# ChainBreak/denoising_diffusion_deep_fake

Measured on AMD Instinct MI355X. Metric: training images/sec (256x256 U-Net, bs=16/GPU), higher is better.
Workload: dtype f32; 1 GPU; d3f train_denoiser step: noise blend -> Unet(resnet34) fwd -> (MSE+1-SSIM)/2 -> bwd -> Adam, 256x256 synthetic face crops, bs=16/GPU, random-init weights, train-mode BatchNorm; image_size=256, batch_per_gpu=16, global_batch=16, parallelism=dp1, graph_step=False, adam_overlap_tail=False, adam_overlap_tail_steps=0, ranks_seen=1, csrc_digest=56899a78a27ce7a0

## Files before the change

### denoising_diffusion_deep_fake_amd/_lib.py

```python
import ctypes as C
import os
import re
from pathlib import Path

_HERE = Path(__file__).resolve().parent
LIB_PATH = Path(os.environ["D3F_LIB"]) if os.environ.get("D3F_LIB") else _HERE / "csrc" / "libd3f_hip.so"
HEADER_PATH = _HERE.parent / "include" / "d3f_hip.h"

F32, BF16, F32X3 = 0, 1, 2


class D3FError(RuntimeError):
    pass


class ConvDesc(C.Structure):
    _fields_ = [(n, C.c_int32) for n in
                ("B", "H", "W", "C0", "C1", "upsample0", "Cout", "KH", "KW", "stride", "pad", "CinReal")]


class BnDesc(C.Structure):
    _fields_ = [("dtype", C.c_int32), ("C", C.c_int32), ("Cpad", C.c_int32), ("rows", C.c_int64),
                ("apply", C.c_int32), ("relu", C.c_int32), ("res", C.c_int32), ("mask", C.c_int32),
                ("fwd_rows", C.c_int32), ("fused_rows", C.c_int32), ("allow_fused", C.c_int32), ("plan_nets", C.c_int32)]


class BnPlan(C.Structure):
    _fields_ = [("fwd_fused", C.c_int32), ("bwd_fused", C.c_int32), ("reduce_blocks", C.c_int32), ("bwd_rows", C.c_int32),
                ("rows_per_block", C.c_int64), ("stat_floats", C.c_uint64), ("part_floats", C.c_uint64)]


BN_COEF_ROWS = 7

_p, _i, _i64, _f, _sz, _dbl = C.c_void_p, C.c_int, C.c_int64, C.c_float, C.c_size_t, C.c_double
_u64, _u32p = C.c_uint64, C.POINTER(C.c_uint32)
_desc = C.POINTER(ConvDesc)
_bnd, _bnp = C.POINTER(BnDesc), C.POINTER(BnPlan)

PROTOTYPES = {
    "d3f_version": (_i, []),
    "d3f_last_error": (C.c_char_p, []),
    "d3f_source_digest": (C.c_char_p, []),
    "d3f_profile_enable": (_i, [_i]),
    "d3f_profile_classes": (_i, [_i]),
    "d3f_profile_collect": (_i, [C.POINTER(C.c_double), C.POINTER(C.c_int64), C.POINTER(C.c_double)]),
    "d3f_unet_create": (_i, [C.c_char_p, _i, _i, _i, _i, _i, _i, C.POINTER(_p)]),
    "d3f_unet_destroy": (_i, [_p]),
    "d3f_unet_create_nets": (_i, [C.c_char_p, _i, _i, _i, _i, _i, _i, _i, _i, C.POINTER(_p)]),
    "d3f_unet_nets": (_i, [_p]),
    "d3f_unet_net_workspace_stride": (_sz, [_p]),
    "d3f_unet_pair_pack_weights": (_i, [_p, C.POINTER(_p), _p, _p]),
    "d3f_unet_pair_forward": (_i, [_p, C.POINTER(_p), C.POINTER(_p), C.POINTER(_p), C.POINTER(_p), _p, _p]),
    "d3f_unet_pair_backward": (_i, [_p, C.POINTER(_p), C.POINTER(_p), C.POINTER(_p), _p, _i, _i, _i, _p]),
    "d3f_unet_num_params": (_i, [_p]),
    "d3f_unet_param_info": (_i, [_p, _i, C.c_char_p, _i, C.POINTER(C.c_int32), C.POINTER(_i), C.POINTER(_i64)]),
    "d3f_unet_param_floats": (_i64, [_p]),
    "d3f_unet_num_bn": (_i, [_p]),
    "d3f_unet_bn_info": (_i, [_p, _i, C.c_char_p, _i, C.POINTER(_i), C.POINTER(_i64), C.POINTER(_i64)]),
    "d3f_unet_bnstat_floats": (_i64, [_p]),
    "d3f_unet_workspace_bytes": (_sz, [_p]),
    "d3f_unet_forward_flops": (_dbl, [_p]),
    "d3f_unet_backward_flops": (_dbl, [_p]),
    "d3f_unet_pack_weights": (_i, [_p, _p, _p, _p]),
    "d3f_unet_forward": (_i, [_p, _p, _p, _p, _p, _p, _i, _p]),
    "d3f_unet_forward_graph": (_i, [_p, _p, _p, _p, _p, _p, _p]),
    "d3f_noise_blend_fixed": (_i, [_p, _p, _p, _p, _i, _i64, _p]),
    "d3f_l1_per_image_workspace_bytes": (_sz, [_i]),
    "d3f_l1_per_image": (_i, [_p, _p, _p, _p, _i, _i64, _p]),
    "d3f_affine_warp": (_i, [_p, _p, _p, _i, _i, _i, _i, _p]),
    "d3f_u8rgb_normalise": (_i, [_p, _p, _i, _i, _i, C.POINTER(_f), C.POINTER(_f), _p]),
    "d3f_unet_predict_u8": (_i, [_p, _p, _p, _p, _p, C.POINTER(_f), C.POINTER(_f), _p, _i, _p]),
    "d3f_unet_predict_frames_u8": (_i, [_p, _p, _p, _p, _i, _i, _i, _i, _i, _i, _p, C.POINTER(_f), C.POINTER(_f), _p, _i, _p]),
    "d3f_crop_resize_cubic_u8": (_i, [_p, _i, _i, _i, _i, _i, _i, _i, _p, _i, _i, _i64, _p]),
    "d3f_unet_num_segments": (_i, [_p]),
    "d3f_unet_plan_counts": (_i, [_p, C.POINTER(C.c_int32), C.POINTER(C.c_int32), C.POINTER(C.c_int32)]),
    "d3f_unet_segment_range": (_i, [_p, _i, C.POINTER(_i64), C.POINTER(_i64)]),
    "d3f_unet_backward": (_i, [_p, _p, _p, _p, _p, _i, _i, _p]),
    "d3f_unet_backward_nojoin": (_i, [_p, _p, _p, _p, _p, _i, _i, _p]),
    "d3f_unet_side_stream": (_i, [_p, C.POINTER(_p)]),
    "d3f_unet_backward_join": (_i, [_p, _p]),
    "d3f_adam_coefficients": (_i, [_f, _f, _f, _f, _i, _f, C.POINTER(_f)]),
    "d3f_unet_train_step": (_i, [_p, _p, _f, _f, _f, _p, _i, _p]),
    "d3f_unet_set_bn_sync": (_i, [_p, _p, _p, _i]),
    "d3f_unet_export": (_i, [_p, C.c_char_p, _p, _p, _p]),
    "d3f_unet_export_shape": (_i, [_p, C.c_char_p, C.POINTER(C.c_int32)]),
    "d3f_conv_upsample_folded": (_i, [_i, _p]),
    "d3f_conv_upsample_summed": (_i, [_i, _p]),
    "d3f_conv_packed_bytes": (_sz, [_i, _desc, _i]),
    "d3f_conv_pack_weights": (_i, [_i, _desc, _p, _p, _p, _p]),
    "d3f_conv_workspace_bytes": (_sz, [_i, _desc, _i]),
    "d3f_conv_stats_floats": (_sz, [_i, _desc, _i, C.POINTER(_i)]),
    "d3f_conv_forward": (_i, [_i, _desc, _p, _p, _p, _p, _p, _p, _p]),
    "d3f_conv_winograd_applies": (_i, [_i, _desc]),
    "d3f_conv_winograd_filter_bytes": (_sz, [_desc]),
    "d3f_conv_winograd_stats_floats": (_sz, [_desc, C.POINTER(_i)]),
    "d3f_conv_winograd_pack": (_i, [_desc, _p, _p, _p]),
    "d3f_conv_winograd_forward": (_i, [_desc, _p, _p, _p, _p, _p, _p, _p, _i, _p]),
    "d3f_conv_backward_data": (_i, [_i, _desc, _p, _p, _p, _p, _i, _i, _p, _p]),
    "d3f_conv_backward_weight_workspace_bytes": (_sz, [_i, _desc]),
    "d3f_conv_backward_weight": (_i, [_i, _desc, _p, _p, _p, _p, _p, _p]),
    "d3f_bn_finalize": (_i, [_p, _i, _i, _i64, _p, _p, _p, _p, _p, _p]),
    "d3f_bn_apply": (_i, [_i, _p, _p, _i, _i64, _p, _i, _p, _p]),
    "d3f_bn_backward_workspace_bytes": (_sz, [_i, _i, _i64]),
    "d3f_bn_backward": (_i, [_i, _p, _p, _p, _p, _p, _i, _i64, _p, _p, _p, _p, _p, _p]),
    "d3f_bn_layer_plan": (_i, [_bnd, _bnp]),
    "d3f_bn_layer_forward": (_i, [_bnd, _p, _p, _p, _p, _p, _p, _p, _p, _p, _p, _p]),
    "d3f_bn_layer_backward": (_i, [_bnd, _p, _p, _p, _p, _p, _p, _p, _p, _i, _p, _p, _p]),
    "d3f_unet_bn_layer": (_i, [_p, _i, _bnd, _bnp]),
    "d3f_maxpool3x3s2_forward": (_i, [_i, _p, _p, _p, _i, _i, _i, _i, _p]),
    "d3f_maxpool3x3s2_backward": (_i, [_i, _p, _p, _p, _i, _i, _i, _i, _i, _p]),
    "d3f_upsample2x_backward": (_i, [_i, _p, _p, _i, _i, _i, _i, _p]),
    "d3f_nchw_to_nhwc": (_i, [_i, _p, _p, _i, _i, _i, _i, _i, _p]),
    "d3f_nhwc_to_nchw": (_i, [_i, _p, _p, _i, _i, _i, _i, _i, _p]),
    "d3f_noise_blend": (_i, [_p, _p, _p, _f, _p, _p, _i, _i64, _p]),
    "d3f_mse_ssim_loss_workspace_bytes": (_sz, [_i, _i, _i]),
    "d3f_mse_ssim_loss": (_i, [_p, _p, _f, _f, _p, _p, _p, _i, _i, _i, _p]),
    "d3f_adam_step": (_i, [_p, _p, _p, _p, _i64, _f, _f, _f, _f, _i, _f, _p]),
    "d3f_ema_lerp": (_i, [_p, _p, _i64, _f, _p]),
    "d3f_philox4x32_10": (_i, [_u32p, _u32p, _u32p]),
    "d3f_noise_blend_rng": (_i, [_p, _u64, _u64, _f, _p, _p, _i, _i64, _p]),
    "d3f_noise_blend_fixed_rng": (_i, [_p, _u64, _u64, _p, _p, _i, _i64, _p]),
    "d3f_noise_draw": (_i, [_u64, _u64, _p, _p, _i, _i64, _p]),
    "d3f_affine_warp_rng": (_i, [_p, _p, _u64, _u64, _i, C.POINTER(_f), _i, _i, _i, _i, _p]),
    "d3f_affine_theta_draw": (_i, [_u64, _u64, _i, C.POINTER(_f), _p, _p, _i, _i, _i, _p]),
}

ALLREDUCE_FN = C.CFUNCTYPE(C.c_int, C.c_void_p, C.c_void_p, C.c_int64, C.c_void_p)

_lib = None


def header_symbols():
    text = HEADER_PATH.read_text()
    text = re.sub(r"/\*.*?\*/", "", text, flags=re.S)
    return sorted(set(re.findall(r"\b(d3f_[a-z0-9_]+)\s*\(", text)))


def sources_present():
    return HEADER_PATH.exists() and any((_HERE / "csrc").glob("*.hip"))


def source_digest():
    import hashlib
    h = hashlib.sha256()
    files = sorted((_HERE / "csrc").glob("*.hip")) + sorted((_HERE / "csrc").glob("*.h")) + [HEADER_PATH]
    for f in files:
        h.update(f.name.encode())
        h.update(f.read_bytes())
    return h.hexdigest()[:16]


def lib():
    global _lib
    if _lib is not None:
        return _lib
    if not LIB_PATH.exists():
        raise D3FError(
            f"{LIB_PATH} is missing: build it with `python -c 'import __graft_entry__ as g; g.build()'` "
            f"or `make -C {LIB_PATH.parent}` (hipcc, gfx950). There is no CPU fallback.")
    handle = C.CDLL(str(LIB_PATH))
    for name, (res, args) in PROTOTYPES.items():
        if os.environ.get("D3F_LIB") and not hasattr(handle, name):
            continue
        fn = getattr(handle, name)
        fn.restype = res
        fn.argtypes = args
    if not os.environ.get("D3F_LIB") and sources_present():
        built, here = handle.d3f_source_digest().decode(), source_digest()
        if built != here:
            raise D3FError(
                f"{LIB_PATH} was built from other sources (digest {built}) than the ones next to it ({here}): "
                f"rebuild it with `make -C {LIB_PATH.parent}`, or name a variant build explicitly through D3F_LIB")
    _lib = handle
    return _lib


def built_digest():
    handle = lib()
    return handle.d3f_source_digest().decode() if hasattr(handle, "d3f_source_digest") else None


def check(rc):
    if rc != 0:
        raise D3FError(lib().d3f_last_error().decode("utf-8", "replace"))


def stream_ptr():
    import torch
    return C.c_void_p(torch.cuda.current_stream().cuda_stream)


def ptr(t):
    if t is None:
        return None
    return C.c_void_p(t.data_ptr())


def ptr2(a, b):
    return (C.c_void_p * 2)(a.data_ptr(), b.data_ptr())
```

### denoising_diffusion_deep_fake_amd/csrc/c_api.hip

```cpp
#include "../../include/d3f_hip.h"

#include <cstdarg>
#include <cstdio>
#include <cstring>
#include <new>
#include <vector>

#include "engine.h"
#include "philox.h"

namespace d3f {
static thread_local char g_err[1024] = "";
int set_error(int code, const char* fmt, ...) {
  va_list ap;
  va_start(ap, fmt);
  vsnprintf(g_err, sizeof(g_err), fmt, ap);
  va_end(ap);
  return code;
}
}

namespace d3f {
struct ProfRec {
  hipEvent_t a, b;
// ... 214 lines not shown
}

int d3f_unet_num_segments(d3f_unet_t h) { return h ? h->e.num_segments : -1; }
int d3f_unet_plan_counts(d3f_unet_t h, int32_t fwd[16], int32_t dgrad[16], int32_t wgrad[16]) {
  D3F_CHECK(h && fwd && dgrad && wgrad, "unet_plan_counts: null argument");
  for (int i = 0; i < 16; ++i) fwd[i] = dgrad[i] = wgrad[i] = 0;
  auto slot = [](int id) { return id < 0 ? 0 : id > 14 ? 14 : id; };
  for (const Unit& u : h->e.units) {
    ++fwd[u.wino ? 15 : slot(u.fwd.patch)];
    if (u.need_dgrad) {
      if (u.upfold) {
        ++dgrad[slot(u.dgrad_lo.patch)];
        if (u.C1 > 0) ++dgrad[slot(u.dgrad.patch)];
      } else {
        ++dgrad[slot(u.dgrad.patch)];
      }
    }
    for (int i = 0; i < u.wl.nparts; ++i) ++wgrad[slot(u.wl.part[i].patch)];
  }
  return 0;
}
int d3f_unet_segment_range(d3f_unet_t h, int segment, int64_t* begin, int64_t* end) {
  D3F_CHECK(h && segment >= 0 && segment < h->e.num_segments, "segment_range: segment %d", segment);
  *begin = h->e.seg_grad_begin[segment];
  *end = h->e.seg_grad_end[segment];
  return 0;
}
int d3f_unet_backward(d3f_unet_t h, const float* params, const float* grad_out, float* grads,
                      void* workspace, int seg_begin, int seg_end, void* stream) {
  D3F_CHECK(h && params && grad_out && grads && workspace, "unet_backward: null argument");
  if (int rc = single_net(h, "unet_backward", "takes d3f_unet_pair_backward")) return rc;
  D3F_CHECK(seg_begin >= 0 && seg_end <= h->e.num_segments && seg_begin <= seg_end,
            "unet_backward: segments [%d,%d)", seg_begin, seg_end);
  return h->e.backward(params, grad_out, grads, workspace, seg_begin, seg_end, (hipStream_t)stream);
}
int d3f_unet_backward_nojoin(d3f_unet_t h, const float* params, const float* grad_out, float* grads,
                             void* workspace, int seg_begin, int seg_end, void* stream) {
  D3F_CHECK(h && params && grad_out && grads && workspace, "unet_backward_nojoin: null argument");
  if (int rc = single_net(h, "unet_backward_nojoin", "takes d3f_unet_pair_backward(join = 0)")) return rc;
  D3F_CHECK(seg_begin >= 0 && seg_end <= h->e.num_segments && seg_begin <= seg_end,
            "unet_backward_nojoin: segments [%d,%d)", seg_begin, seg_end);
  return h->e.backward(params, grad_out, grads, workspace, seg_begin, seg_end, (hipStream_t)stream, 0);
}
int d3f_unet_side_stream(d3f_unet_t h, void** stream_out) {
  D3F_CHECK(h && stream_out, "unet_side_stream: null argument");
  *stream_out = (void*)h->e.side_stream();
  return 0;
}
int d3f_unet_backward_join(d3f_unet_t h, void* stream) {
  D3F_CHECK(h, "unet_backward_join: null handle");
  return h->e.backward_join((hipStream_t)stream);
}
int d3f_adam_coefficients(float lr, float beta1, float beta2, float eps, int step, float grad_scale, float coef[8]) {
  D3F_CHECK(coef && step >= 1, "adam_coefficients: step counts from 1");
  adam_coefficients(lr, beta1, beta2, eps, step, grad_scale, coef);
  return 0;
}
int d3f_unet_train_step(d3f_unet_t h, const d3f_step_buffers* b, float lam, float input_min, float input_max,
                        void* workspace, int use_graph, void* stream) {
  D3F_CHECK(h && b && workspace, "unet_train_step: null argument");
  if (int rc = single_net(h, "unet_train_step", "has no captured step (d3f_unet_pair_forward / _backward, then per network)"))
    return rc;
  D3F_CHECK(b->params && b->bnstats && b->grads && b->exp_avg && b->exp_avg_sq && b->image && b->noise && b->y_uniform &&
                b->noisy && b->pred && b->grad_pred && b->loss_out && b->loss_workspace && b->adam_coef,
            "unet_train_step: null buffer");
  D3F_CHECK(!h->e.bn_sync_installed(),
            "unet_train_step: synchronised BatchNorm statistics call back into the host inside the pass; the captured "
            "step is the single-GPU form (use forward / backward)");
  UnetEngine::StepArgs a;
  std::memset(&a, 0, sizeof(a));
  a.params = b->params; a.bnstats = b->bnstats; a.grads = b->grads; a.exp_avg = b->exp_avg; a.exp_avg_sq = b->exp_avg_sq;
  a.image = b->image; a.noise = b->noise; a.y_uniform = b->y_uniform;
  a.noisy = b->noisy; a.pred = b->pred; a.gpred = b->grad_pred; a.loss_out = b->loss_out;
  a.loss_ws = reinterpret_cast<float*>(b->loss_workspace);
  a.adam_coef = b->adam_coef;
  a.lam = lam; a.lo = input_min; a.hi = input_max;
  return h->e.train_step(a, workspace, use_graph, (hipStream_t)stream);
}
int d3f_unet_set_bn_sync(d3f_unet_t h, d3f_allreduce_fn fn, void* ctx, int world_size) {
  D3F_CHECK(h && (fn == nullptr || world_size >= 1), "unet_set_bn_sync: arguments");
  if (fn != nullptr) {
    if (int rc = single_net(h, "unet_set_bn_sync", "keeps per-GPU BatchNorm statistics")) return rc;
  }
  h->e.set_bn_sync(fn, ctx, world_size);
  return 0;
}
int d3f_unet_export(d3f_unet_t h, const char* name, const void* workspace, float* out_nchw, void* stream) {
  D3F_CHECK(h && name && workspace && out_nchw, "unet_export: null argument");
  return h->e.export_tensor(name, workspace, out_nchw, (hipStream_t)stream);
}
int d3f_unet_export_shape(d3f_unet_t h, const char* name, int32_t dims[3]) {
  D3F_CHECK(h && name && dims, "unet_export_shape: null argument");
  return h->e.export_shape(name, dims);
}

size_t d3f_conv_packed_bytes(int dtype, const d3f_conv_desc* d, int which) {
  ConvLayer L;
  if (plan(L, dtype, d, 0) != 0) return 0;
  if (L.upfold) return which == 0 ? L.wfc : L.wd4 + L.wds;
  return which == 0 ? L.wf : L.wd;
}
int d3f_conv_pack_weights(int dtype, const d3f_conv_desc* d, const float* w, void* w_fwd, void* w_dgrad,
                          void* stream) {
  ConvLayer L;
  if (int rc = plan(L, dtype, d, 0)) return rc;
  if (L.upfold) {
    D3F_CHECK(w_fwd != nullptr && d->CinReal == d->C0 + d->C1, "conv_pack_weights: up-sample folded layer");
    char* wds = w_dgrad && d->C1 > 0 ? reinterpret_cast<char*>(w_dgrad) + L.wd4 : nullptr;
    return pack_up_launch(dtype, w, d->Cout, d->C0, d->C1, w_fwd, L.CoutPad, w_dgrad, L.C0Rows, wds, L.C1Rows,
                          (hipStream_t)stream);
  }
  void* const dst[2] = {w_fwd, w_dgrad};
  PackTable t[2];
  int blocks[2] = {0, 0};
  for (int k = 0; k < 2; ++k) {
    t[k].n = dst[k] != nullptr ? 1 : 0;
    if (t[k].n && (blocks[k] = conv_pack_entry(L, 0, 0, 0, k == 0, k == 1, 0, t[k].e[0])) < 0) return blocks[k];
  }
  for (int k = 0; k < 2; ++k)
    if (int rc = pack_all_launch(dtype, w, dst[k], t[k], blocks[k], (hipStream_t)stream)) return rc;
  return 0;
}
int d3f_conv_upsample_folded(int dtype, const d3f_conv_desc* d) {
  ConvLayer L;
  return (d != nullptr && plan(L, dtype, d, 0) == 0 && L.upfold) ? 1 : 0;
}
int d3f_conv_upsample_summed(int dtype, const d3f_conv_desc* d) {
  ConvLayer L, D;
  if (d == nullptr || !d->upsample0 || plan(L, dtype, d, 0) != 0 || L.upfold) return 0;
  return (plan(D, dtype, d, PLAN_DGRAD | PLAN_SUM2) == 0 && D.dgrad.sum2) ? 1 : 0;
}
size_t d3f_conv_workspace_bytes(int dtype, const d3f_conv_desc* d, int which) {
  ConvLayer L;
  const int what = which == 0 ? PLAN_FWD : PLAN_DGRAD | (d != nullptr && d->upsample0 == 2 ? PLAN_SUM2 : 0);
  return plan(L, dtype, d, what | PLAN_SPLITK) != 0 ? 0 : L.splitk_floats * sizeof(float);
}
size_t d3f_conv_stats_floats(int dtype, const d3f_conv_desc* d, int with_workspace, int* tiles) {
  ConvLayer L;
  if (plan(L, dtype, d, PLAN_FWD | (with_workspace ? PLAN_SPLITK : 0)) != 0) return 0;
  if (tiles) *tiles = L.fwd.stat_rows;
  return (size_t)L.fwd.stat_rows * L.CoutPad * 2;
}
int d3f_conv_forward(int dtype, const d3f_conv_desc* d, const void* src0, const void* src1,
                     const void* w_fwd, void* y, float* stats, void* workspace, void* stream) {
  ConvLayer L;
  if (int rc = plan(L, dtype, d, PLAN_FWD | (workspace ? PLAN_SPLITK : 0))) return rc;
  if (d->B == 0) return 0;
  D3F_CHECK(src0 && w_fwd && y && (d->C1 == 0 || src1), "conv_forward: null argument");
  ConvFwdBufs b;
  b.src0 = src0; b.src1 = src1; b.w = w_fwd; b.out = y; b.stats = stats;
  b.slabs = reinterpret_cast<float*>(workspace);
  return conv_layer_forward(L, b, false, (hipStream_t)stream);
}
static int wino_plan(ConvLayer& L, const d3f_conv_desc* d) {
  if (int rc = plan(L, D3F_F32, d, PLAN_FWD)) return rc;
  D3F_CHECK(L.wu != 0,
            "conv_winograd: needs 3x3 / stride 1 / pad 1, one source, H and W multiples of 16, channels a multiple of 16, "
            "filters a multiple of 64 (got %dx%d k%d s%d p%d C0=%d C1=%d up=%d Cout=%d)",
            d->H, d->W, d->KH, d->stride, d->pad, d->C0, d->C1, d->upsample0, d->Cout);
  return 0;
}
int d3f_conv_winograd_applies(int dtype, const d3f_conv_desc* d) {
  ConvLayer L;
  return (d != nullptr && plan(L, dtype, d, PLAN_FWD) == 0 && L.wino) ? 1 : 0;
}
size_t d3f_conv_winograd_filter_bytes(const d3f_conv_desc* d) {
  ConvLayer L;
  return (d == nullptr || plan(L, D3F_F32, d, PLAN_FWD) != 0) ? 0 : L.wu;
}
size_t d3f_conv_winograd_stats_floats(const d3f_conv_desc* d, int* tiles) {
  ConvLayer L;
  if (d == nullptr || plan(L, D3F_F32, d, PLAN_FWD) != 0 || L.wu == 0) return 0;
  if (tiles) *tiles = L.wino_rows;
  return (size_t)L.wino_rows * L.CoutPad * 2;
}
int d3f_conv_winograd_pack(const d3f_conv_desc* d, const float* w, void* u, void* stream) {
  ConvLayer L;
  if (int rc = wino_plan(L, d)) return rc;
  D3F_CHECK(w && u && d->CinReal == d->C0, "conv_winograd_pack: null argument or padded input channels");
  return conv_winograd_pack_launch(w, reinterpret_cast<float*>(u), d->Cout, d->C0, (hipStream_t)stream);
}
int d3f_conv_winograd_forward(const d3f_conv_desc* d, const void* src0, const void* u, void* y, float* stats,
                              const float* scale, const float* shift, const void* residual, int relu, void* stream) {
  ConvLayer L;
  if (int rc = wino_plan(L, d)) return rc;
  if (d->B == 0) return 0;
  D3F_CHECK(src0 && u && y && ((scale == nullptr) == (shift == nullptr)), "conv_winograd_forward: null argument");
  D3F_CHECK(scale != nullptr || (residual == nullptr && relu == 0),
            "conv_winograd_forward: residual / ReLU belong to the eval epilogue (scale and shift)");
  ConvFwdBufs b;
  b.src0 = src0; b.w = u; b.out = y;
  if (scale != nullptr) {
    b.scale = scale; b.shift = shift; b.res = residual; b.relu = relu ? 1 : 0;
  } else {
    b.stats = stats;
  }
  return conv_layer_forward(L, b, true, (hipStream_t)stream);
}
int d3f_conv_backward_data(int dtype, const d3f_conv_desc* d, const void* dy, const void* w_dgrad,
                           void* dx0, void* dx1, int acc0, int acc1, void* workspace, void* stream) {
  ConvLayer L;
  const int sum2 = d != nullptr && d->upsample0 == 2 ? PLAN_SUM2 : 0;
  if (int rc = plan(L, dtype, d, PLAN_DGRAD | sum2 | (workspace ? PLAN_SPLITK : 0))) return rc;
  if (d->B == 0) return 0;
  D3F_CHECK(dy && w_dgrad && dx0 && (d->C1 == 0 || dx1), "conv_backward_data: null argument");
  ConvDgradBufs b;
  b.dy = dy; b.w = w_dgrad; b.dx0 = dx0; b.dx1 = dx1; b.acc0 = acc0; b.acc1 = acc1;
  b.w_skip = L.upfold ? reinterpret_cast<const char*>(w_dgrad) + L.wd4 : nullptr;
  b.slabs = reinterpret_cast<float*>(workspace);
  return conv_layer_dgrad(L, b, (hipStream_t)stream);
}
size_t d3f_conv_backward_weight_workspace_bytes(int dtype, const d3f_conv_desc* d) {
  ConvLayer L;
  return plan(L, dtype, d, PLAN_WGRAD) != 0 ? 0 : L.wslab_bytes;
}
int d3f_conv_backward_weight(int dtype, const d3f_conv_desc* d, const void* dy, const void* src0,
                             const void* src1, void* workspace, float* dw, void* stream) {
  ConvLayer L;
  if (int rc = plan(L, dtype, d, PLAN_WGRAD)) return rc;
  if (d->B == 0) {
    D3F_CHECK(dw, "conv_backward_weight: null argument");
    D3F_HIP(hipMemsetAsync(dw, 0, (size_t)d->Cout * d->CinReal * d->KH * d->KW * sizeof(float), (hipStream_t)stream));
    return 0;
  }
  D3F_CHECK(dy && src0 && workspace && dw && (d->C1 == 0 || src1), "conv_backward_weight: null argument");
  return wgrad_layer_launch(L.wl, dy, src0, src1, reinterpret_cast<float*>(workspace), dw, d->Cout, d->CinReal, dtype,
                            (hipStream_t)stream);
}

static BnLayer bn_layer(int dtype, int C, int64_t rows, int fwd_rows = 0) {
  BnLayer L;
  L.C = C; L.Cpad = (int)round_up(C, 16); L.rows = (long)rows; L.dtype = sdt(dtype); L.fwd_rows = fwd_rows;
  L.allow_fused = false;
  bn_layer_plan(L);
  return L;
}
int d3f_bn_finalize(const float* stats, int tiles, int C, int64_t count, const float* gamma,
                    const float* beta, float* running_mean, float* running_var, float* coef, void* stream) {
  D3F_CHECK(stats && gamma && beta && coef && C > 0 && tiles > 0 && count > 0, "bn_finalize: argument");
  const BnLayer L = bn_layer(D3F_F32, C, count, tiles);
  BnBufs b;
  b.stats = const_cast<float*>(stats);
  b.gamma = gamma; b.beta = beta; b.running_mean = running_mean; b.running_var = running_var; b.coef = coef;
  return bn_layer_finalize(L, b, (long)count, (hipStream_t)stream);
}
int d3f_bn_apply(int dtype, const void* y, const float* coef, int C, int64_t rows, const void* residual,
                 int relu, void* out, void* stream) {
  D3F_CHECK(y && coef && out, "bn_apply: null argument");
  BnLayer L = bn_layer(dtype, C, rows);
  L.relu = relu != 0;
  L.res = residual ? BN_RES_TENSOR : BN_RES_NONE;
  BnBufs b;
  b.coef = const_cast<float*>(coef);
  b.y = y; b.res = residual; b.a = out;
  return bn_layer_apply(L, b, (hipStream_t)stream);
}
size_t d3f_bn_backward_workspace_bytes(int dtype, int C, int64_t rows) {
  return ((size_t)bn_layer(dtype, C, rows).reduce_blocks * C * 2 + 3 * (size_t)C) * sizeof(float) + 256;
}
int d3f_bn_backward(int dtype, const void* dA, const void* a_or_null, const void* y, const float* coef,
                    const float* gamma, int C, int64_t rows, void* dy, void* dres, float* dgamma,
                    float* dbeta, void* workspace, void* stream) {
  D3F_CHECK(dA && y && coef && gamma && dy && dgamma && dbeta && workspace, "bn_backward: null argument");
  BnLayer L = bn_layer(dtype, C, rows);
  L.mask = a_or_null ? BN_MASK_FROM_A : BN_MASK_NONE;
  BnBufs b;
  b.stats = reinterpret_cast<float*>(workspace);
  b.k = b.stats + (size_t)round_up((long)L.reduce_blocks * C * 2, 4);
  b.coef = const_cast<float*>(coef);
  b.gamma = gamma; b.y = y; b.a = const_cast<void*>(a_or_null);
  b.dA = dA; b.dy = dy; b.dres = dres; b.dgamma = dgamma; b.dbeta = dbeta;
  return bn_layer_backward(L, b, nullptr, (hipStream_t)stream);
}

static_assert(D3F_BN_COEF_ROWS == BN_COEF_ROWS, "d3f_hip.h states the coefficient block's rows");
static int bn_plan(BnLayer& L, const d3f_bn_desc* d) {
  D3F_CHECK(d != nullptr, "bn_layer: null descriptor");
  D3F_CHECK(d->dtype == D3F_F32 || d->dtype == D3F_BF16 || d->dtype == D3F_F32X3, "bn_layer: dtype %d", d->dtype);
  D3F_CHECK(d->C > 0 && d->Cpad >= d->C && d->rows >= 0, "bn_layer: C=%d Cpad=%d rows=%lld", d->C, d->Cpad,
            (long long)d->rows);
  D3F_CHECK(d->res >= BN_RES_NONE && d->res <= BN_RES_LAYER && d->mask >= BN_MASK_NONE && d->mask <= BN_MASK_FROM_A,
            "bn_layer: res=%d mask=%d", d->res, d->mask);
  D3F_CHECK(d->fwd_rows >= 0 && d->fused_rows >= 0, "bn_layer: fwd_rows=%d fused_rows=%d", d->fwd_rows, d->fused_rows);
  D3F_CHECK(d->plan_nets == 1 || d->plan_nets == 2, "bn_layer: plan_nets=%d", d->plan_nets);
  L.name = "bn_layer";
  L.C = d->C; L.Cpad = d->Cpad; L.rows = (long)d->rows; L.dtype = sdt(d->dtype); L.plan_nets = d->plan_nets;
  L.apply = d->apply != 0; L.relu = d->relu != 0;
  L.res = (BnResidual)d->res; L.mask = (BnMask)d->mask;
  L.fwd_rows = d->fwd_rows; L.fused_rows = d->fused_rows; L.allow_fused = d->allow_fused != 0;
  bn_layer_plan(L);
  return 0;
}
static void bn_plan_out(const BnLayer& L, d3f_bn_plan* p) {
  p->fwd_fused = L.fwd_fused; p->bwd_fused = L.bwd_fused; p->reduce_blocks = L.reduce_blocks; p->bwd_rows = L.bwd_rows;
  p->rows_per_block = L.rows_per_block; p->stat_floats = L.stat_floats; p->part_floats = L.part_floats;
}
static bool bn_split_channels_ok(const BnLayer& L) {
  const int ve = L.dtype == D3F_F32 ? 4 : 8;
  return L.C % ve == 0 && (256 * ve) % L.C == 0;
}
int d3f_bn_layer_plan(const d3f_bn_desc* d, d3f_bn_plan* plan) {
  D3F_CHECK(plan != nullptr, "bn_layer_plan: null argument");
  BnLayer L;
  if (int rc = bn_plan(L, d)) return rc;
  bn_plan_out(L, plan);
  return 0;
}
int d3f_bn_layer_forward(const d3f_bn_desc* d, float* stats, const float* gamma, const float* beta, float* running_mean,
                         float* running_var, float* coef, const void* y, const void* res, const float* res_coef, void* a,
                         void* stream) {
  BnLayer L;
  if (int rc = bn_plan(L, d)) return rc;
  if (L.rows == 0) return 0;
  D3F_CHECK(L.fwd_rows >= 1, "bn_layer_forward: the forward pass reads fwd_rows >= 1 partial rows (fwd_rows=%d)", L.fwd_rows);
  D3F_CHECK(stats && gamma && beta && coef && y, "bn_layer_forward: null argument");
  D3F_CHECK((running_mean == nullptr) == (running_var == nullptr), "bn_layer_forward: one running statistic without the other");
  if (L.apply) {
    D3F_CHECK(a != nullptr, "bn_layer_forward: apply needs the output tensor");
    D3F_CHECK(L.res == BN_RES_NONE || res != nullptr, "bn_layer_forward: res=%d needs the residual tensor", (int)L.res);
    D3F_CHECK(L.res != BN_RES_LAYER || res_coef != nullptr, "bn_layer_forward: res=2 needs res_coef, the other layer's coefficient block");
  }
  if (L.fwd_fused)
    D3F_CHECK(L.Cpad % 2 == 0, "bn_layer_forward: the fused form needs an even Cpad (Cpad=%d)", L.Cpad);
  else if (L.apply)
    D3F_CHECK(bn_split_channels_ok(L), "bn_layer_forward: the split form needs C to divide %d (C=%d)",
              256 * (L.dtype == D3F_F32 ? 4 : 8), L.C);
  BnBufs b;
  b.stats = stats; b.gamma = gamma; b.beta = beta; b.running_mean = running_mean; b.running_var = running_var;
  b.coef = coef; b.y = y; b.a = a; b.res = res; b.res_coef = res_coef;
  return bn_layer_forward(L, b, nullptr, (hipStream_t)stream);
}
int d3f_bn_layer_backward(const d3f_bn_desc* d, float* partial, const float* gamma, float* coef, const void* y,
                          const void* a, const void* dA, void* dy, void* dres, int dres_acc, float* dgamma, float* dbeta,
                          void* stream) {
  BnLayer L;
  if (int rc = bn_plan(L, d)) return rc;
  if (L.rows == 0) return 0;
  D3F_CHECK(partial != nullptr, "bn_layer_backward: null partial rows (fused_rows=%d: %s)", L.fused_rows,
            L.fused_rows > 0 ? "the caller's sums" : "scratch of part_floats floats");
  D3F_CHECK(gamma && coef && y && dA && dy, "bn_layer_backward: null argument");
  D3F_CHECK(L.mask != BN_MASK_FROM_A || a != nullptr, "bn_layer_backward: mask=2 needs the activation a");
  D3F_CHECK((dgamma == nullptr) == (dbeta == nullptr), "bn_layer_backward: dgamma without dbeta or the reverse");
  if (L.fused_rows == 0 || !L.bwd_fused)
    D3F_CHECK(bn_split_channels_ok(L), "bn_layer_backward: the split kernels need C to divide %d (C=%d)",
              256 * (L.dtype == D3F_F32 ? 4 : 8), L.C);
  BnBufs b;
  b.stats = partial; b.gamma = gamma; b.coef = coef; b.y = y;
  b.a = const_cast<void*>(a);
  b.dA = dA; b.dy = dy; b.dres = dres; b.dres_acc = dres != nullptr && dres_acc ? 1 : 0;
  b.dgamma = dgamma; b.dbeta = dbeta;
  return bn_layer_backward(L, b, nullptr, (hipStream_t)stream);
}
int d3f_unet_bn_layer(d3f_unet_t h, int i, d3f_bn_desc* d, d3f_bn_plan* plan) {
  D3F_CHECK(h && d && plan && i >= 0 && i < (int)h->e.bns.size(), "bn_layer: index %d", i);
  int k = -1;
  for (const Unit& u : h->e.units) {
    if (!u.bn || ++k != i) continue;
    const BnLayer& L = u.norm;
    d->dtype = L.dtype; d->C = L.C; d->Cpad = L.Cpad; d->rows = L.rows; d->apply = L.apply; d->relu = L.relu;
    d->res = L.res; d->mask = L.mask; d->fwd_rows = L.fwd_rows; d->fused_rows = L.fused_rows;
    d->allow_fused = L.allow_fused; d->plan_nets = L.plan_nets;
    bn_plan_out(L, plan);
// ... 139 lines not shown
```

### denoising_diffusion_deep_fake_amd/csrc/common.h

```cpp
#pragma once
#include <hip/hip_runtime.h>
#include <stdint.h>
#include <stddef.h>
#include <stdlib.h>

namespace d3f {

typedef uint16_t bf16_t;

typedef float f32x16 __attribute__((ext_vector_type(16)));
typedef float f32x4 __attribute__((ext_vector_type(4)));
typedef __bf16 bf16x8 __attribute__((ext_vector_type(8)));

}
#ifndef D3F_F32
#define D3F_F32 0
#define D3F_BF16 1
#define D3F_F32X3 2
#endif
namespace d3f {

static inline const char* prof_knob(const char* name) {
#ifdef D3F_PROFILING
  return getenv(name);
#else
  (void)name;
  return nullptr;
#endif
}

int set_error(int code, const char* fmt, ...);
#define D3F_CHECK(cond, ...)                              \
  do {                                                    \
    if (!(cond)) return ::d3f::set_error(-1, __VA_ARGS__); \
  } while (0)
#define D3F_HIP(expr)                                                                 \
  do {                                                                                \
    hipError_t e_ = (expr);                                                           \
    if (e_ != hipSuccess)                                                             \
      return ::d3f::set_error(-2, "%s failed: %s (%s:%d)", #expr, hipGetErrorString(e_), \
                              __FILE__, __LINE__);                                    \
  } while (0)

__device__ __forceinline__ float bf16_to_f32(bf16_t v) {
  return __uint_as_float(((uint32_t)v) << 16);
}
__device__ __forceinline__ bf16_t f32_to_bf16(float f) {
  __bf16 b = (__bf16)f;
  return *reinterpret_cast<bf16_t*>(&b);
}
template <typename T> __device__ __forceinline__ float to_f32(T v);
template <> __device__ __forceinline__ float to_f32<float>(float v) { return v; }
template <> __device__ __forceinline__ float to_f32<bf16_t>(bf16_t v) { return bf16_to_f32(v); }
template <typename T> __device__ __forceinline__ T from_f32(float v);
template <> __device__ __forceinline__ float from_f32<float>(float v) { return v; }
template <> __device__ __forceinline__ bf16_t from_f32<bf16_t>(float v) { return f32_to_bf16(v); }

template <typename T> __device__ __forceinline__ float4 ld4(const T* p);
template <> __device__ __forceinline__ float4 ld4<float>(const float* p) { return *reinterpret_cast<const float4*>(p); }
template <> __device__ __forceinline__ float4 ld4<bf16_t>(const bf16_t* p) {
  const uint2 v = *reinterpret_cast<const uint2*>(p);
  return make_float4(__uint_as_float(v.x << 16), __uint_as_float(v.x & 0xffff0000u), __uint_as_float(v.y << 16),
                     __uint_as_float(v.y & 0xffff0000u));
}
template <typename T> __device__ __forceinline__ void st4(T* p, const float4& v);
template <> __device__ __forceinline__ void st4<float>(float* p, const float4& v) { *reinterpret_cast<float4*>(p) = v; }
template <> __device__ __forceinline__ void st4<bf16_t>(bf16_t* p, const float4& v) {
  const uint32_t a = (uint32_t)f32_to_bf16(v.x) | ((uint32_t)f32_to_bf16(v.y) << 16);
  const uint32_t b = (uint32_t)f32_to_bf16(v.z) | ((uint32_t)f32_to_bf16(v.w) << 16);
  *reinterpret_cast<uint2*>(p) = make_uint2(a, b);
}

typedef unsigned int u32x4_t __attribute__((ext_vector_type(4)));
constexpr unsigned BUF_OOB = 0x80000000u;
__device__ __forceinline__ __amdgpu_buffer_rsrc_t make_rsrc(const void* p, unsigned bytes) {
  return __builtin_amdgcn_make_buffer_rsrc(const_cast<void*>(p), 0, (int)bytes, 0x00020000);
}
__device__ __forceinline__ uint4 buf_load16(__amdgpu_buffer_rsrc_t r, unsigned byte_off) {
  const u32x4_t v = __builtin_amdgcn_raw_buffer_load_b128(r, (int)byte_off, 0, 0);
  return make_uint4(v.x, v.y, v.z, v.w);
}

__device__ __forceinline__ uint4 buf_load16s(__amdgpu_buffer_rsrc_t r, unsigned byte_off, unsigned soff) {
  const u32x4_t v = __builtin_amdgcn_raw_buffer_load_b128(r, (int)byte_off, (int)soff, 0);
  return make_uint4(v.x, v.y, v.z, v.w);
}

#ifndef D3F_CHAIN_PRIO
#define D3F_CHAIN_PRIO 3
#endif
__device__ __forceinline__ void chain_priority() {
#if D3F_CHAIN_PRIO > 0
  __builtin_amdgcn_s_setprio(D3F_CHAIN_PRIO);
#endif
}

struct NetSplit {
  int nets;
  long ws;
  long par;
  long grad;
  long bn;
  long in;
  long out;
};
static inline int nets_of(int n) { return n > 1 ? n : 1; }
static inline int plan_nets_for(int plan_nets, int bit) {
  static const int mask = prof_knob("D3F_PLAN_MASK") ? atoi(prof_knob("D3F_PLAN_MASK")) : -1;
  return (mask & bit) ? nets_of(plan_nets) : 1;
}
static inline NetSplit net_split_or_single(const NetSplit* ns) {
  NetSplit one{};
  one.nets = 1;
  return (ns != nullptr && ns->nets > 1) ? *ns : one;
}
template <typename P> __device__ __forceinline__ void net_shift(P& p, long bytes) {
  if (p != nullptr) p = reinterpret_cast<P>(reinterpret_cast<uintptr_t>(p) + bytes);
}

template <typename T> struct Elem;
template <> struct Elem<float> {
  static constexpr int VE = 4;
  static constexpr int BKE = 32;
};
template <> struct Elem<bf16_t> {
  static constexpr int VE = 8;
  static constexpr int BKE = 64;
};

static inline void fast_div_setup(unsigned d, unsigned* mul, unsigned* shr) {
  if (d <= 1) { *mul = 0; *shr = 0; return; }
  unsigned lg = 0;
  while ((1ull << lg) < d) ++lg;
  const unsigned p = 31 + lg;
  *mul = (unsigned)(((1ull << p) + d - 1) / d);
  *shr = p - 32;
}
__device__ __forceinline__ int fast_div(int n, unsigned mul, unsigned shr) {
  return mul ? (int)(__umulhi((unsigned)n, mul) >> shr) : n;
}

static inline int cdiv(long a, long b) { return (int)((a + b - 1) / b); }
static inline long round_up(long a, long b) { return (a + b - 1) / b * b; }

enum ProfClass : int { PROF_CONV_FWD = 0, PROF_CONV_DGRAD = 1, PROF_WGRAD = 2, PROF_NUM = 3 };
bool prof_enabled(int cls);
void prof_begin(int cls, double flops, hipStream_t s);
void prof_end(hipStream_t s);

enum ConvMode : int {
  CONV_RAW_STATS = 0,
  CONV_HEAD_NCHW = 1,
  CONV_EVAL_FUSED = 2,
  CONV_DGRAD = 3,
};

struct ConvParams {
  const void* src0;
  const void* src1;
  const void* w;
  void* out0;
  void* out1;
  float* stats;
  const float* scale;
  const float* shift;
  const void* res;
  unsigned src0_bytes, src1_bytes, w_bytes;
  int B, Hv, Wv;
  int C0, C1;
  int H0s, W0s;
  int shift0;
  int zi;
  int Ho, Wo, Cout;
  int CoutPad, Kpad;
  int w_ld;
  int par;
  int nz;
  int KH, KW, stride, pad;
  int M;
  int tiles_m, tiles_n;
  float* partial;
  int splitk;
  int stat_rows;
  int out_c0;
  int acc0, acc1;
  int mode;
  int relu;
  double flops;
  const void* bn_y;
  const float* bn_coef;
  float* bn_partial;
  const void* bn_a;
  unsigned div_howo_mul, div_howo_shr, div_wo_mul, div_wo_shr;
  int cin_real;
  int sum2;
  int patch;
  int nets, plan_nets;
  long net_ws, net_out0, net_scale;
  int tile_bm, tile_bn;
};
__device__ __forceinline__ ConvParams conv_params_of_net(const ConvParams& pin, int net) {
  ConvParams p = pin;
  if (net != 0) {
    net_shift(p.src0, p.net_ws); net_shift(p.src1, p.net_ws); net_shift(p.w, p.net_ws);
    net_shift(p.out0, p.net_out0); net_shift(p.out1, p.net_ws);
    net_shift(p.stats, p.net_ws); net_shift(p.scale, p.net_scale); net_shift(p.shift, p.net_ws);
    net_shift(p.res, p.net_ws); net_shift(p.partial, p.net_ws);
    net_shift(p.bn_y, p.net_ws); net_shift(p.bn_coef, p.net_ws); net_shift(p.bn_partial, p.net_ws); net_shift(p.bn_a, p.net_ws);
  }
  return p;
}

struct ConvTile {
  int BM, BN;
};
int conv_igemm_plan(ConvParams& p, int dtype, bool allow_splitk = false);
size_t conv_splitk_floats(const ConvParams& p);
int conv_igemm_launch(const ConvParams& p, int dtype, hipStream_t stream);
bool conv_winograd_fits(const ConvParams& p, int dtype);
bool conv_winograd_applies(const ConvParams& p, int dtype);
int conv_winograd_stat_rows(const ConvParams& p);
size_t conv_winograd_filter_floats(const ConvParams& p);
int conv_winograd_pack_launch(const float* w , float* u, int Cout, int Cin, hipStream_t stream);
int conv_winograd_launch(const ConvParams& p , hipStream_t stream);
bool conv_pres_applies(const ConvParams& p, int dtype);
void conv_pres_plan(ConvParams& p);
int conv_pres_launch(const ConvParams& p, hipStream_t stream);
bool conv_patch_applies(const ConvParams& p, int dtype);
bool conv_stem_applies(const ConvParams& p, int dtype);
bool conv_stem_bf16_applies(const ConvParams& p, int dtype);
void conv_patch_plan(ConvParams& p, int dtype);
int conv_patch_launch(const ConvParams& p, hipStream_t stream);

struct WgradParams {
  const void* dy;
  const void* src0;
  const void* src1;
  float* partial;
  unsigned dy_bytes, src0_bytes, src1_bytes;
  int B, Hv, Wv, C0, C1, H0s, W0s, shift0;
  int Ho, Wo, Cout;
  int KH, KW, stride, pad;
  int M;
  int cin_real;
  int splits;
  int chunks_per_split;
  int tiles_co, tiles_ci;
  int patch;
  double flops;
  int part;
  int cls;
  int ci_base;
  int slab_cin;
  int slab_taps;
  int Mi, Hc, Wc;
  int step_img, step_row, step_col;
  int nets, plan_nets;
  long net_ws;
};
__device__ __forceinline__ WgradParams wgrad_params_of_net(const WgradParams& pin, int net) {
  WgradParams p = pin;
  if (net != 0) {
    net_shift(p.dy, p.net_ws); net_shift(p.src0, p.net_ws); net_shift(p.src1, p.net_ws); net_shift(p.partial, p.net_ws);
  }
  return p;
}
enum WgradPart : int { WG_WHOLE = 0, WG_CLASS = 1, WG_SKIP = 2 };
int wgrad_plan(WgradParams& p, int dtype);
size_t wgrad_partial_floats(const WgradParams& p);
int wgrad_launch(const WgradParams& p, int dtype, hipStream_t stream);

constexpr int WG_BATCH = 20;
struct WgradReduceJob {
  const float* partial;
  float* dw;
  int splits, CoutP, Cin, CinReal, taps, CB, nsg, VB, CinTot, c_off, fold, Cout, cz, block0, lds;
};
struct WgradReduceBatch {
  WgradReduceJob job[WG_BATCH];
  int n = 0, blocks = 0, lds = 0;
  int nets = 1;
  long net_ws = 0, net_grad = 0;
};
int wgrad_reduce_batch_add(WgradReduceBatch& tb, const float* partial, int splits, int CoutP, int Cout, int Cin,
                           int CinRealPart, int CinRealTotal, int c_off, int KH, int KW, int fold, float* dw);
int wgrad_reduce_batch_launch(const WgradReduceBatch& tb, hipStream_t stream);

struct WgradLayer {
  WgradParams part[2];
  int nparts;
};
int wgrad_layer_plan(WgradLayer& L, const WgradParams& base, int dtype);
size_t wgrad_layer_partial_floats(const WgradLayer& L);
int wgrad_layer_launch(const WgradLayer& L, const void* dy, const void* src0, const void* src1, float* partial,
                       float* dw, int CoutReal, int CinReal, int dtype, hipStream_t stream);
int wgrad_layer_launch_deferred(const WgradLayer& L, const void* dy, const void* src0, const void* src1, float* partial,
                                float* dw, int CoutReal, int CinReal, int dtype, WgradReduceBatch& tb,
                                hipStream_t stream, const NetSplit* ns = nullptr);

struct ConvLayer {
  int B = 0, Hv = 0, Wv = 0;
  int C0 = 0, C1 = 0, up0 = 0;
  int CinReal = 0, Cout = 0, KH = 0, KW = 0, stride = 1, pad = 0;
  int dtype = 0;
  bool head = false;
  bool need_fwd = false, need_dgrad = false, need_wgrad = false;
  bool want_sum2 = false;
  bool allow_splitk = false;
  int plan_nets = 0;
  int sdtype = 0;
  int Cin = 0, Ho = 0, Wo = 0, CoutPad = 0, Kpad = 0, CoutD = 0, KpadD = 0, CinRows = 0, C0Rows = 0, C1Rows = 0;
  bool upfold = false;
  bool parity = false;
  bool wino = false;
  ConvParams fwd{}, dgrad{}, dgrad_lo{};
  WgradLayer wl{};
  int wino_rows = 0;
  size_t wf = 0, wd = 0;
  size_t wfc = 0, wd4 = 0, wds = 0;
  size_t wu = 0;
  size_t splitk_floats = 0;
  size_t wslab_bytes = 0;
  double macs = 0;
};
int conv_layer_plan(ConvLayer& L);

struct ConvFwdBufs {
  const void* src0 = nullptr;
  const void* src1 = nullptr;
  const void* w = nullptr;
  void* out = nullptr;
  float* stats = nullptr;
  const float* bias = nullptr;
  const float* scale = nullptr;
  const float* shift = nullptr;
  const void* res = nullptr;
  int relu = 0;
  float* slabs = nullptr;
};
int conv_layer_forward(const ConvLayer& L, const ConvFwdBufs& b, bool wino, hipStream_t s, const NetSplit* ns = nullptr);
struct ConvDgradBufs {
  const void* dy = nullptr;
  const void* w = nullptr;
  const void* w_skip = nullptr;
  void* dx0 = nullptr;
  void* dx1 = nullptr;
  int acc0 = 0, acc1 = 0;
  float* slabs = nullptr;
  const void* bn_y = nullptr;
  const float* bn_coef = nullptr;
  float* bn_partial = nullptr;
  const void* bn_a = nullptr;
};
int conv_layer_dgrad(const ConvLayer& L, const ConvDgradBufs& b, hipStream_t s, const NetSplit* ns = nullptr);
struct PackEntry;
int conv_pack_entry(const ConvLayer& L, long w_off, size_t wf_off, size_t wd_off, bool fwd, bool dgrad, uint32_t block0,
                    PackEntry& e);

}
```

### denoising_diffusion_deep_fake_amd/csrc/conv_patch.hip

```cpp
#include "common.h"

#include <cstdlib>

namespace d3f {

constexpr int CP_PH = 4, CP_PW = 64;

static bool patch_conv_off() {
  static const bool off = getenv("D3F_NO_PATCH_CONV") != nullptr;
  return off;
}

bool conv_patch_applies(const ConvParams& p, int dtype) {
  if (patch_conv_off() || (dtype != D3F_F32 && dtype != D3F_BF16)) return false;
  const bool mode_ok = p.mode == CONV_RAW_STATS || p.mode == CONV_HEAD_NCHW ||
                       (p.mode == CONV_EVAL_FUSED && p.res == nullptr) ||
                       (p.mode == CONV_DGRAD && p.out_c0 == p.Cout && (p.Cout % 4) == 0);
  const bool wide = p.C0 == 32 && dtype == D3F_BF16 && p.mode != CONV_HEAD_NCHW;
  const bool cin_ok = p.C0 == 16 || wide || (p.C0 == 4 && p.mode == CONV_DGRAD && dtype == D3F_F32) ||
                      (p.C0 == 8 && p.mode == CONV_DGRAD && dtype == D3F_BF16);
  const bool up = wide && p.shift0 == 1 && p.mode != CONV_DGRAD && p.Cout <= 16 && p.H0s * 2 == p.Hv && p.W0s * 2 == p.Wv;
  const bool sum2 = p.sum2 && dtype == D3F_BF16 && p.mode == CONV_DGRAD && p.C0 == 16 && p.Cout == 32 && p.shift0 == 0;
  if (p.sum2 && !sum2) return false;
  return mode_ok && p.par == 0 && p.KH == 3 && p.KW == 3 && p.stride == 1 && p.pad == 1 && cin_ok && p.C1 == 0 &&
         (p.shift0 == 0 || up) && p.zi == 0 && p.Cout <= (wide && !up ? 64 : sum2 ? 32 : 16) && (p.mode == CONV_HEAD_NCHW || (p.Cout % 4) == 0) &&
         p.Hv == p.Ho && p.Wv == p.Wo && (p.Ho % CP_PH) == 0 &&
         (p.Wo % CP_PW) == 0 && p.Kpad >= 9 * p.C0;
}

template <typename T, int CIN, int BN, bool UP = false, int CSRC = CIN, bool SUM2 = false>
__global__ __launch_bounds__(256) void conv_patch_kernel(const ConvParams pin) {
  const ConvParams p = conv_params_of_net(pin, (int)blockIdx.z);
  chain_priority();
  constexpr bool BF = sizeof(T) == 2;
  constexpr bool W64 = BF && CIN == 32;
  static_assert(!UP || (W64 && BN == 16), "up-sampled source: bf16 x 32 channels -> 16 filters");
  static_assert(CSRC == CIN || (BF && CIN == 16 && CSRC == 8 && !UP), "half-filled pixels: bf16, 8 of 16 channels");
  static_assert(!SUM2 || (BF && CIN == 16 && CSRC == 16 && BN == 32 && !UP), "2x2-summed data gradient: bf16 x 16 -> 32");
  static_assert(((CIN == 16 || (CIN == 4 && !BF)) && (BN == 16 || SUM2)) || (W64 && (BN == 32 || UP)),
                "16 channels (forward / data gradient of decoder block 4, head forward), fp32 x 4 (data gradient of the "
                "head) or bf16 x 32 -> 32 (decoder block 3 conv2)");
  constexpr int VEC = 16 / (int)sizeof(T);
  constexpr int PH = CP_PH, PW = CP_PW, PR = UP ? PH / 2 + 2 : PH + 2, PC = UP ? PW / 2 + 2 : PW + 2;
  constexpr int CS = W64 ? 20 : BF ? 10 : (CIN == 16 ? CIN + 4 : 12);
  constexpr int KR = 9 * CIN;
  constexpr int WS = W64 ? KR / 2 : BF ? KR / 2 + 2 : (CIN == 16 ? KR : KR + 4);
  constexpr int CV = CSRC / VEC;
  constexpr int KS = 9 * CSRC;
  constexpr int NPV = PR * PC * CV;
  constexpr int NWV = BN * (KS / VEC);
  constexpr int NLP = (NPV + 255) / 256, NLW = (NWV + 255) / 256;
  constexpr int BM = PH * PW, LDC = BN + 4, FM = PW / 16, NB = BN / 16;
  constexpr int PATCH_DW = PR * PC * CS > BM * LDC ? PR * PC * CS : BM * LDC;
  __shared__ __attribute__((aligned(16))) float lds[PATCH_DW + BN * WS];
  float* P = lds;
  float* Wl = lds + PATCH_DW;

  const int tid = threadIdx.x, lane = tid & 63, wave = tid >> 6;
  const int tiles_x = p.Wo / PW, tiles_y = p.Ho / PH;
  const int tile = (int)blockIdx.x;
  const int tx = tile % tiles_x, ty = (tile / tiles_x) % tiles_y, b = tile / (tiles_x * tiles_y);
  const int y0 = ty * PH, x0 = tx * PW;
  const int n0 = (int)blockIdx.y * BN;

  const __amdgpu_buffer_rsrc_t rs = make_rsrc(p.src0, p.src0_bytes);
  const __amdgpu_buffer_rsrc_t rw = make_rsrc(p.w, p.w_bytes);
  uint4 pv[NLP], wv[NLW];
#pragma unroll
  for (int i = 0; i < NLP; ++i) {
    const int id = tid + 256 * i;
    const int pix = id / CV, cv = id - pix * CV;
    const int pr = pix / PC, pc = pix - pr * PC;
    const int gy = (UP ? y0 / 2 : y0) - 1 + pr, gx = (UP ? x0 / 2 : x0) - 1 + pc;
    const int Hs = UP ? p.H0s : p.Hv, Ws = UP ? p.W0s : p.Wv;
    const bool ok = id < NPV && (unsigned)gy < (unsigned)Hs && (unsigned)gx < (unsigned)Ws;
    pv[i] = buf_load16(rs, ok ? (unsigned)(((b * Hs + gy) * Ws + gx) * CSRC + cv * VEC) * (unsigned)sizeof(T) : BUF_OOB);
  }
#pragma unroll
  for (int i = 0; i < NLW; ++i) {
    const int id = tid + 256 * i;
    const int row = id / (KS / VEC), ch = id - row * (KS / VEC);
    const bool ok = id < NWV && n0 + row < p.CoutPad;
    wv[i] = buf_load16(rw, ok ? (unsigned)((n0 + row) * p.w_ld + ch * VEC) * (unsigned)sizeof(T) : BUF_OOB);
  }
#pragma unroll
  for (int i = 0; i < NLP; ++i) {
    const int id = tid + 256 * i;
    const int pix = id / CV, cv = id - pix * CV;
    if (NPV % 256 == 0 || id < NPV) {
      if constexpr (BF && !W64) {
        *reinterpret_cast<uint2*>(&P[pix * CS + cv * 4]) = make_uint2(pv[i].x, pv[i].y);
        *reinterpret_cast<uint2*>(&P[pix * CS + cv * 4 + 2]) = make_uint2(pv[i].z, pv[i].w);
        if constexpr (CSRC < CIN) {
          *reinterpret_cast<uint2*>(&P[pix * CS + 4]) = make_uint2(0u, 0u);
          *reinterpret_cast<uint2*>(&P[pix * CS + 6]) = make_uint2(0u, 0u);
        }
      } else {
        *reinterpret_cast<uint4*>(&P[pix * CS + cv * 4]) = pv[i];
      }
    }
  }
#pragma unroll
  for (int i = 0; i < NLW; ++i) {
    const int id = tid + 256 * i;
    const int row = id / (KS / VEC), ch = id - row * (KS / VEC);
    if (NWV % 256 == 0 || id < NWV) {
      if constexpr (CSRC < CIN) {
        *reinterpret_cast<uint2*>(&Wl[row * WS + ch * 8]) = make_uint2(wv[i].x, wv[i].y);
        *reinterpret_cast<uint2*>(&Wl[row * WS + ch * 8 + 2]) = make_uint2(wv[i].z, wv[i].w);
        *reinterpret_cast<uint2*>(&Wl[row * WS + ch * 8 + 4]) = make_uint2(0u, 0u);
        *reinterpret_cast<uint2*>(&Wl[row * WS + ch * 8 + 6]) = make_uint2(0u, 0u);
      } else if constexpr (BF && !W64) {
        *reinterpret_cast<uint2*>(&Wl[row * WS + ch * 4]) = make_uint2(wv[i].x, wv[i].y);
        *reinterpret_cast<uint2*>(&Wl[row * WS + ch * 4 + 2]) = make_uint2(wv[i].z, wv[i].w);
      } else {
        const int chs = (CIN == 16 || W64) ? (ch ^ ((row >> 1) & 3)) : ch;
        *reinterpret_cast<uint4*>(&Wl[row * WS + chs * 4]) = wv[i];
      }
    }
  }
  __syncthreads();

  const int fr = lane & 15, fq = lane >> 4;
  f32x4 acc[FM * NB];
#pragma unroll
  for (int i = 0; i < FM * NB; ++i) acc[i] = f32x4{0.f, 0.f, 0.f, 0.f};
  if constexpr (UP) {
    const float* Bbase = Wl + fr * WS + (fq ^ ((fr >> 1) & 3)) * 4;
    const float* Acol[3];
#pragma unroll
    for (int kw = 0; kw < 3; ++kw) Acol[kw] = P + (((fr + kw - 1) >> 1) + 1) * CS + fq * 4;
#pragma unroll
    for (int tap = 0; tap < 9; ++tap) {
      const int kh = tap / 3, kw = tap - kh * 3;
      const int prow = ((wave + kh - 1) >> 1) + 1;
      const uint4 bb = *reinterpret_cast<const uint4*>(Bbase + tap * (CIN / 2));
      uint4 a[FM];
#pragma unroll
      for (int i = 0; i < FM; ++i) a[i] = *reinterpret_cast<const uint4*>(Acol[kw] + (prow * PC + 8 * i) * CS);
#pragma unroll
      for (int i = 0; i < FM; ++i)
        acc[i] = __builtin_amdgcn_mfma_f32_16x16x32_bf16(*reinterpret_cast<const bf16x8*>(&a[i]),
                                                         *reinterpret_cast<const bf16x8*>(&bb), acc[i], 0, 0, 0);
    }
  } else if constexpr (W64) {
    const float* Abase = P + (wave * PC + fr) * CS + fq * 4;
    const float* Bbase = Wl + fr * WS + (fq ^ ((fr >> 1) & 3)) * 4;
#pragma unroll
    for (int tap = 0; tap < 9; ++tap) {
      const int kh = tap / 3, kw = tap - kh * 3;
      uint4 bb[NB], a[FM];
#pragma unroll
      for (int j = 0; j < NB; ++j) bb[j] = *reinterpret_cast<const uint4*>(Bbase + j * 16 * WS + tap * (CIN / 2));
#pragma unroll
      for (int i = 0; i < FM; ++i) a[i] = *reinterpret_cast<const uint4*>(Abase + ((kh * PC + kw) + i * 16) * CS);
#pragma unroll
      for (int i = 0; i < FM; ++i)
#pragma unroll
        for (int j = 0; j < NB; ++j)
          acc[i * NB + j] = __builtin_amdgcn_mfma_f32_16x16x32_bf16(*reinterpret_cast<const bf16x8*>(&a[i]),
                                                                    *reinterpret_cast<const bf16x8*>(&bb[j]), acc[i * NB + j], 0, 0, 0);
    }
  } else if constexpr (BF) {
    typedef short v4s __attribute__((ext_vector_type(4)));
    const float* Abase = P + (wave * PC + fr) * CS + fq * 2;
    const float* Bbase = Wl + fr * WS + fq * 2;
#pragma unroll
    for (int tap = 0; tap < 9; ++tap) {
      const int kh = tap / 3, kw = tap - kh * 3;
      v4s bb[NB];
#pragma unroll
      for (int j = 0; j < NB; ++j) bb[j] = *reinterpret_cast<const v4s*>(Bbase + j * 16 * WS + tap * (CIN / 2));
#pragma unroll
      for (int i = 0; i < FM; ++i) {
        const v4s a = *reinterpret_cast<const v4s*>(Abase + ((kh * PC + kw) + i * 16) * CS);
#pragma unroll
        for (int j = 0; j < NB; ++j) acc[i * NB + j] = __builtin_amdgcn_mfma_f32_16x16x16bf16_1k(a, bb[j], acc[i * NB + j], 0, 0, 0);
      }
    }
  } else if constexpr (CIN == 16) {
    const float* Abase = P + (wave * PC + fr) * CS + fq * 4;
    const float* Bbase = Wl + fr * WS + (fq ^ ((fr >> 1) & 3)) * 4;
#pragma unroll
    for (int tap = 0; tap < 9; ++tap) {
      const int kh = tap / 3, kw = tap - kh * 3;
      const uint4 bb = *reinterpret_cast<const uint4*>(Bbase + tap * CIN);
      uint4 a[FM];
#pragma unroll
      for (int i = 0; i < FM; ++i)
        a[i] = *reinterpret_cast<const uint4*>(Abase + ((kh * PC + kw) + i * 16) * CS);
#pragma unroll
      for (int i = 0; i < FM; ++i) acc[i] = __builtin_amdgcn_mfma_f32_16x16x4f32(__uint_as_float(a[i].x), __uint_as_float(bb.x), acc[i], 0, 0, 0);
#pragma unroll
      for (int i = 0; i < FM; ++i) acc[i] = __builtin_amdgcn_mfma_f32_16x16x4f32(__uint_as_float(a[i].y), __uint_as_float(bb.y), acc[i], 0, 0, 0);
#pragma unroll
      for (int i = 0; i < FM; ++i) acc[i] = __builtin_amdgcn_mfma_f32_16x16x4f32(__uint_as_float(a[i].z), __uint_as_float(bb.z), acc[i], 0, 0, 0);
#pragma unroll
      for (int i = 0; i < FM; ++i) acc[i] = __builtin_amdgcn_mfma_f32_16x16x4f32(__uint_as_float(a[i].w), __uint_as_float(bb.w), acc[i], 0, 0, 0);
    }
  } else {
    const float* Abase = P + (wave * PC + fr) * CS + fq;
    const float* Bbase = Wl + fr * WS + fq;
#pragma unroll
    for (int tap = 0; tap < 9; ++tap) {
      const int kh = tap / 3, kw = tap - kh * 3;
      const float bb = Bbase[tap * CIN];
      float a[FM];
#pragma unroll
      for (int i = 0; i < FM; ++i) a[i] = Abase[((kh * PC + kw) + i * 16) * CS];
#pragma unroll
      for (int i = 0; i < FM; ++i) acc[i] = __builtin_amdgcn_mfma_f32_16x16x4f32(a[i], bb, acc[i], 0, 0, 0);
    }
  }

  const int HoWo = p.Ho * p.Wo;
  const long mrow0 = ((long)b * p.Ho + y0) * p.Wo + x0;
  if (NB == 1 && p.mode == CONV_HEAD_NCHW) {
    if (fr < p.Cout) {
      float* __restrict__ out = reinterpret_cast<float*>(p.out0);
      const float bias = p.scale ? p.scale[fr] : 0.f;
      float* orow = out + ((long)b * p.Cout + fr) * HoWo + (long)(y0 + wave) * p.Wo + x0 + 4 * fq;
#pragma unroll
      for (int i = 0; i < FM; ++i)
        *reinterpret_cast<float4*>(orow + 16 * i) =
            make_float4(acc[i][0] + bias, acc[i][1] + bias, acc[i][2] + bias, acc[i][3] + bias);
    }
    return;
  }
// ... 89 lines not shown
    if (n_ok) {
#pragma unroll
      for (int i = 0; i < NVEC; ++i) {
        const int row = rv0 + i * RSTEP;
        st4<T>(out + out_row(row) * p.Cout + n, *reinterpret_cast<const float4*>(&Cs[row * LDC + cv * 4]));
      }
    }
    if (p.stats != nullptr) {
      constexpr int NG = 256 / BN;
      const int col = tid % BN, rg = tid / BN;
      float s1 = 0.f, s2 = 0.f;
      for (int row = rg; row < BM; row += NG) {
        const float v = Cs[row * LDC + col];
        s1 += v;
        s2 += v * v;
      }
      __syncthreads();
      float* red = lds;
      red[(rg * BN + col) * 2 + 0] = s1;
      red[(rg * BN + col) * 2 + 1] = s2;
      __syncthreads();
      if (tid < BN) {
        float a1 = 0.f, a2 = 0.f;
#pragma unroll
        for (int g = 0; g < NG; ++g) {
          a1 += red[(g * BN + tid) * 2 + 0];
          a2 += red[(g * BN + tid) * 2 + 1];
        }
        if (n0 + tid < p.CoutPad) {
          p.stats[((long)tile * p.CoutPad + n0 + tid) * 2 + 0] = a1;
          p.stats[((long)tile * p.CoutPad + n0 + tid) * 2 + 1] = a2;
        }
      }
    }
  } else if (p.mode == CONV_EVAL_FUSED) {
    T* __restrict__ out = reinterpret_cast<T*>(p.out0);
    if (n_ok) {
      const float4 sc = *reinterpret_cast<const float4*>(p.scale + n), sf = *reinterpret_cast<const float4*>(p.shift + n);
#pragma unroll
      for (int i = 0; i < NVEC; ++i) {
        const int row = rv0 + i * RSTEP;
        float4 v = *reinterpret_cast<const float4*>(&Cs[row * LDC + cv * 4]);
        v.x = v.x * sc.x + sf.x; v.y = v.y * sc.y + sf.y; v.z = v.z * sc.z + sf.z; v.w = v.w * sc.w + sf.w;
        if (p.relu) { v.x = fmaxf(v.x, 0.f); v.y = fmaxf(v.y, 0.f); v.z = fmaxf(v.z, 0.f); v.w = fmaxf(v.w, 0.f); }
        st4<T>(out + out_row(row) * p.Cout + n, v);
      }
    }
  } else {
    T* __restrict__ o0 = reinterpret_cast<T*>(p.out0);
    if (n_ok) {
#pragma unroll
      for (int i = 0; i < NVEC; ++i) {
        const int row = rv0 + i * RSTEP;
        float4 v = *reinterpret_cast<const float4*>(&Cs[row * LDC + cv * 4]);
        T* dst = o0 + out_row(row) * p.Cout + n;
        if (p.acc0) {
          const float4 o = ld4<T>(dst);
          v.x += o.x; v.y += o.y; v.z += o.z; v.w += o.w;
          if (p.bn_partial != nullptr) *reinterpret_cast<float4*>(&Cs[row * LDC + cv * 4]) = v;
        }
        st4<T>(dst, v);
      }
    }
    if (p.bn_partial != nullptr) {
      const int C = p.Cout;
      const T* __restrict__ yb = reinterpret_cast<const T*>(p.bn_y);
      const T* __restrict__ ab = reinterpret_cast<const T*>(p.bn_a);
      float s1[4] = {0.f, 0.f, 0.f, 0.f}, s2[4] = {0.f, 0.f, 0.f, 0.f};
      if (n_ok) {
        const float4 mu = *reinterpret_cast<const float4*>(p.bn_coef + n), is = *reinterpret_cast<const float4*>(p.bn_coef + C + n);
        const float4 sc = *reinterpret_cast<const float4*>(p.bn_coef + 2 * C + n), sf = *reinterpret_cast<const float4*>(p.bn_coef + 3 * C + n);
        const float m4[4] = {mu.x, mu.y, mu.z, mu.w}, i4[4] = {is.x, is.y, is.z, is.w};
        const float c4[4] = {sc.x, sc.y, sc.z, sc.w}, f4[4] = {sf.x, sf.y, sf.z, sf.w};
        float4 yv[NVEC], av[NVEC];
#pragma unroll
        for (int i = 0; i < NVEC; ++i) {
          const long m = out_row(rv0 + i * RSTEP);
          yv[i] = ld4<T>(yb + m * C + n);
          av[i] = ab != nullptr ? ld4<T>(ab + m * C + n) : make_float4(0.f, 0.f, 0.f, 0.f);
        }
#pragma unroll
        for (int i = 0; i < NVEC; ++i) {
          const float4 gv = *reinterpret_cast<const float4*>(&Cs[(rv0 + i * RSTEP) * LDC + cv * 4]);
          const float yy[4] = {yv[i].x, yv[i].y, yv[i].z, yv[i].w}, aa[4] = {av[i].x, av[i].y, av[i].z, av[i].w};
          const float gg[4] = {gv.x, gv.y, gv.z, gv.w};
#pragma unroll
          for (int k = 0; k < 4; ++k) {
            const float keep = ab != nullptr ? aa[k] : yy[k] * c4[k] + f4[k];
            const float g = keep > 0.f ? gg[k] : 0.f;
            s1[k] += g;
            s2[k] += g * ((yy[k] - m4[k]) * i4[k]);
          }
        }
      }
      __syncthreads();
      float* red = lds;
#pragma unroll
      for (int k = 0; k < 4; ++k) {
        red[(rv0 * BN + cv * 4 + k) * 2 + 0] = s1[k];
        red[(rv0 * BN + cv * 4 + k) * 2 + 1] = s2[k];
      }
      __syncthreads();
      if (tid < BN) {
        float a1 = 0.f, a2 = 0.f;
#pragma unroll 8
        for (int g = 0; g < RSTEP; ++g) {
          a1 += red[(g * BN + tid) * 2 + 0];
          a2 += red[(g * BN + tid) * 2 + 1];
        }
        if (n0 + tid < C) {
          p.bn_partial[((long)tile * C + n0 + tid) * 2 + 0] = a1;
          p.bn_partial[((long)tile * C + n0 + tid) * 2 + 1] = a2;
        }
      }
    }
  }
}

constexpr int ST_PH = 8, ST_PW = 32, ST_BN = 32;

bool conv_stem_applies(const ConvParams& p, int dtype) {
  if (patch_conv_off() || dtype != D3F_F32) return false;
  const bool mode_ok = (p.mode == CONV_RAW_STATS) || (p.mode == CONV_EVAL_FUSED && p.res == nullptr);
  return mode_ok && p.par == 0 && p.KH == 7 && p.KW == 7 && p.stride == 2 && p.pad == 3 && p.C0 == 4 && p.C1 == 0 &&
         p.shift0 == 0 && p.zi == 0 && (p.Cout % ST_BN) == 0 && p.Hv == 2 * p.Ho && p.Wv == 2 * p.Wo &&
         (p.Ho % ST_PH) == 0 && (p.Wo % ST_PW) == 0 && p.Kpad >= 49 * 4;
}

__global__ __launch_bounds__(256) void conv_stem_kernel(const ConvParams pin) {
  const ConvParams p = conv_params_of_net(pin, (int)blockIdx.z);
  chain_priority();
  constexpr int PH = ST_PH, PW = ST_PW, BN = ST_BN;
  constexpr int PR = 2 * PH + 5, PC = 2 * PW + 5;
  constexpr int NE = (PC + 1) / 2;
  constexpr int PATCH_DW = PR * PC * 4 + 4;
  constexpr int WS = 7 * 4 * 2 * 4 + 4;
  constexpr int NPV = PR * PC, NWV = BN * 56;
  constexpr int NLP = (NPV + 255) / 256, NLW = (NWV + 255) / 256;
  constexpr int BM = PH * PW, LDC = BN + 4;
  static_assert(BM * LDC <= PATCH_DW + BN * WS, "the C tile aliases the staging area");
  __shared__ __attribute__((aligned(16))) float lds[PATCH_DW + BN * WS];
  float* P = lds;
  float* Wl = lds + PATCH_DW;

  const int tid = threadIdx.x, lane = tid & 63, wave = tid >> 6;
  const int tiles_x = p.Wo / PW, tiles_y = p.Ho / PH;
  const int tile = (int)blockIdx.x, n0 = (int)blockIdx.y * BN;
  const int tx = tile % tiles_x, ty = (tile / tiles_x) % tiles_y, b = tile / (tiles_x * tiles_y);
  const int y0 = ty * PH, x0 = tx * PW;

  const __amdgpu_buffer_rsrc_t rs = make_rsrc(p.src0, p.src0_bytes);
  const __amdgpu_buffer_rsrc_t rw = make_rsrc(p.w, p.w_bytes);
  uint4 pv[NLP], wv[NLW];
#pragma unroll
  for (int i = 0; i < NLP; ++i) {
    const int id = tid + 256 * i;
    const int pr = id / PC, pc = id - pr * PC;
    const int gy = 2 * y0 - 3 + pr, gx = 2 * x0 - 3 + pc;
    const bool ok = id < NPV && (unsigned)gy < (unsigned)p.Hv && (unsigned)gx < (unsigned)p.Wv;
    pv[i] = buf_load16(rs, ok ? (unsigned)(((b * p.Hv + gy) * p.Wv + gx) * 4) * 4u : BUF_OOB);
  }
#pragma unroll
  for (int i = 0; i < NLW; ++i) {
    const int id = tid + 256 * i;
    const int n = id / 56, r = id - n * 56, kh = r >> 3, kw = r & 7;
    const bool ok = id < NWV && kw < 7 && (n0 + n) < p.CoutPad;
    wv[i] = buf_load16(rw, ok ? (unsigned)((n0 + n) * p.w_ld + (kh * 7 + kw) * 4) * 4u : BUF_OOB);
  }
#pragma unroll
  for (int i = 0; i < NLP; ++i) {
    const int id = tid + 256 * i;
    const int pr = id / PC, pc = id - pr * PC;
    if (id < NPV) *reinterpret_cast<uint4*>(&P[(pr * PC + (pc & 1) * NE + (pc >> 1)) * 4]) = pv[i];
  }
  if (tid == 0) *reinterpret_cast<uint4*>(&P[PR * PC * 4]) = make_uint4(0u, 0u, 0u, 0u);
#pragma unroll
  for (int i = 0; i < NLW; ++i) {
    const int id = tid + 256 * i;
    const int n = id / 56, r = id - n * 56;
    if (NWV % 256 == 0 || id < NWV) *reinterpret_cast<uint4*>(&Wl[n * WS + r * 4]) = wv[i];
  }
  __syncthreads();

  const int fr = lane & 31, fq = lane >> 5;
  f32x16 acc[2];
#pragma unroll
  for (int i = 0; i < 2; ++i)
#pragma unroll
    for (int r = 0; r < 16; ++r) acc[i][r] = 0.f;
  const float* Abase = P + ((4 * wave) * PC + fq * NE + fr) * 4;
  const float* Bbase = Wl + fr * WS + fq * 4;
#pragma unroll
  for (int kh = 0; kh < 7; ++kh) {
#pragma unroll
    for (int j = 0; j < 4; ++j) {
      const uint4 bb = *reinterpret_cast<const uint4*>(Bbase + (kh * 4 + j) * 8);
      uint4 a[2];
#pragma unroll
      for (int i = 0; i < 2; ++i) a[i] = *reinterpret_cast<const uint4*>(Abase + ((2 * i + kh) * PC + j) * 4);
#pragma unroll
      for (int i = 0; i < 2; ++i) acc[i] = __builtin_amdgcn_mfma_f32_32x32x2f32(__uint_as_float(a[i].x), __uint_as_float(bb.x), acc[i], 0, 0, 0);
#pragma unroll
      for (int i = 0; i < 2; ++i) acc[i] = __builtin_amdgcn_mfma_f32_32x32x2f32(__uint_as_float(a[i].y), __uint_as_float(bb.y), acc[i], 0, 0, 0);
#pragma unroll
      for (int i = 0; i < 2; ++i) acc[i] = __builtin_amdgcn_mfma_f32_32x32x2f32(__uint_as_float(a[i].z), __uint_as_float(bb.z), acc[i], 0, 0, 0);
    }
  }

  __syncthreads();
  float* Cs = lds;
#pragma unroll
  for (int i = 0; i < 2; ++i)
#pragma unroll
    for (int r = 0; r < 16; ++r)
      Cs[((2 * wave + i) * PW + (r & 3) + 8 * (r >> 2) + 4 * fq) * LDC + fr] = acc[i][r];
  __syncthreads();

  constexpr int VN = BN / 4, NVEC = BM * VN / 256, RSTEP = 256 / VN;
  const int cv = tid % VN, rv0 = tid / VN;
  const int n = n0 + cv * 4;
  const long mrow0 = ((long)b * p.Ho + y0) * p.Wo + x0;
  auto out_row = [&](int row) { return mrow0 + (long)(row / PW) * p.Wo + (row % PW); };
  float* __restrict__ out = reinterpret_cast<float*>(p.out0);
  if (p.mode == CONV_RAW_STATS) {
#pragma unroll
    for (int i = 0; i < NVEC; ++i) {
      const int row = rv0 + i * RSTEP;
      *reinterpret_cast<float4*>(out + out_row(row) * p.Cout + n) = *reinterpret_cast<const float4*>(&Cs[row * LDC + cv * 4]);
    }
    if (p.stats != nullptr) {
      constexpr int NG = 256 / BN;
      const int col = tid % BN, rg = tid / BN;
      float s1 = 0.f, s2 = 0.f;
      for (int row = rg; row < BM; row += NG) {
        const float v = Cs[row * LDC + col];
        s1 += v;
        s2 += v * v;
      }
      __syncthreads();
      float* red = lds;
      red[(rg * BN + col) * 2 + 0] = s1;
      red[(rg * BN + col) * 2 + 1] = s2;
      __syncthreads();
      if (tid < BN) {
        float a1 = 0.f, a2 = 0.f;
#pragma unroll
        for (int g = 0; g < NG; ++g) {
          a1 += red[(g * BN + tid) * 2 + 0];
          a2 += red[(g * BN + tid) * 2 + 1];
        }
        p.stats[((long)tile * p.CoutPad + n0 + tid) * 2 + 0] = a1;
        p.stats[((long)tile * p.CoutPad + n0 + tid) * 2 + 1] = a2;
      }
    }
  } else {
    const float4 sc = *reinterpret_cast<const float4*>(p.scale + n), sf = *reinterpret_cast<const float4*>(p.shift + n);
#pragma unroll
    for (int i = 0; i < NVEC; ++i) {
      const int row = rv0 + i * RSTEP;
      float4 v = *reinterpret_cast<const float4*>(&Cs[row * LDC + cv * 4]);
      v.x = v.x * sc.x + sf.x; v.y = v.y * sc.y + sf.y; v.z = v.z * sc.z + sf.z; v.w = v.w * sc.w + sf.w;
      if (p.relu) { v.x = fmaxf(v.x, 0.f); v.y = fmaxf(v.y, 0.f); v.z = fmaxf(v.z, 0.f); v.w = fmaxf(v.w, 0.f); }
      *reinterpret_cast<float4*>(out + out_row(row) * p.Cout + n) = v;
    }
  }
}

bool conv_stem_bf16_applies(const ConvParams& p, int dtype) {
  if (patch_conv_off() || dtype != D3F_BF16) return false;
#ifdef D3F_NO_PATCH32
  return false;
#endif
  const bool mode_ok = (p.mode == CONV_RAW_STATS) || (p.mode == CONV_EVAL_FUSED && p.res == nullptr);
  return mode_ok && p.par == 0 && p.KH == 7 && p.KW == 7 && p.stride == 2 && p.pad == 3 && p.C0 == 8 && p.C1 == 0 &&
         p.cin_real >= 1 && p.cin_real <= 4 &&
         p.shift0 == 0 && p.zi == 0 && (p.Cout % ST_BN) == 0 && p.Hv == 2 * p.Ho && p.Wv == 2 * p.Wo &&
         (p.Ho % ST_PH) == 0 && (p.Wo % ST_PW) == 0 && p.Kpad >= 49 * 8;
}

__global__ __launch_bounds__(256) void conv_stem_bf16_kernel(const ConvParams pin) {
  const ConvParams p = conv_params_of_net(pin, (int)blockIdx.z);
  chain_priority();
  constexpr int PH = ST_PH, PW = ST_PW, BN = ST_BN;
  constexpr int PR = 2 * PH + 5, PC = 2 * PW + 5;
  constexpr int PCS = PC + 3;
  constexpr int PATCH_DW = PR * PCS * 2 + 4;
  constexpr int WS = 7 * 8 * 2 + 4;
  constexpr int NPV = PR * PC, NWV = BN * 49;
  constexpr int NLP = (NPV + 255) / 256, NLW = (NWV + 255) / 256;
  constexpr int BM = PH * PW, LDC = BN + 4;
  constexpr int LDS_DW = BM * LDC > PATCH_DW + BN * WS ? BM * LDC : PATCH_DW + BN * WS;
  __shared__ __attribute__((aligned(16))) float lds[LDS_DW];
  float* P = lds;
  float* Wl = lds + PATCH_DW;

  const int tid = threadIdx.x, lane = tid & 63, wave = tid >> 6;
  const int tiles_x = p.Wo / PW, tiles_y = p.Ho / PH;
  const int tile = (int)blockIdx.x, n0 = (int)blockIdx.y * BN;
  const int tx = tile % tiles_x, ty = (tile / tiles_x) % tiles_y, b = tile / (tiles_x * tiles_y);
  const int y0 = ty * PH, x0 = tx * PW;

  const __amdgpu_buffer_rsrc_t rs = make_rsrc(p.src0, p.src0_bytes);
  const __amdgpu_buffer_rsrc_t rw = make_rsrc(p.w, p.w_bytes);
  uint4 pv[NLP], wv[NLW];
#pragma unroll
  for (int i = 0; i < NLP; ++i) {
    const int id = tid + 256 * i;
    const int pr = id / PC, pc = id - pr * PC;
    const int gy = 2 * y0 - 3 + pr, gx = 2 * x0 - 3 + pc;
    const bool ok = id < NPV && (unsigned)gy < (unsigned)p.Hv && (unsigned)gx < (unsigned)p.Wv;
    pv[i] = buf_load16(rs, ok ? (unsigned)(((b * p.Hv + gy) * p.Wv + gx) * 8) * 2u : BUF_OOB);
  }
#pragma unroll
  for (int i = 0; i < NLW; ++i) {
    const int id = tid + 256 * i;
    const int n = id / 49, t = id - n * 49;
    const bool ok = id < NWV && (n0 + n) < p.CoutPad;
    wv[i] = buf_load16(rw, ok ? (unsigned)((n0 + n) * p.w_ld + t * 8) * 2u : BUF_OOB);
  }
  for (int id = tid; id < PR * 3; id += 256) {
// ... 152 lines not shown
```

### denoising_diffusion_deep_fake_amd/csrc/conv_plan.hip

```cpp
#include "pointwise.h"

#include <algorithm>

namespace d3f {

int conv_layer_plan(ConvLayer& L) {
  D3F_CHECK(L.dtype == D3F_F32 || L.dtype == D3F_BF16 || L.dtype == D3F_F32X3, "conv: dtype %d", L.dtype);
  L.sdtype = L.dtype == D3F_F32X3 ? D3F_F32 : L.dtype;
  const int ve = L.sdtype == D3F_F32 ? 4 : 8, bke = L.sdtype == D3F_F32 ? 32 : 64;
  const size_t wsz = L.dtype == D3F_F32X3 ? 6 : L.sdtype == D3F_F32 ? 4 : 2;
  D3F_CHECK(L.B >= 0 && L.Hv > 0 && L.Wv > 0 && L.C0 > 0 && L.C1 >= 0 && L.Cout > 0, "conv: extent");
  D3F_CHECK(L.C0 % ve == 0 && L.C1 % ve == 0, "conv: channels must be multiples of %d", ve);
  D3F_CHECK(L.KH == L.KW && L.KH >= 1 && L.KH <= 7, "conv: kernel %dx%d", L.KH, L.KW);
  D3F_CHECK(L.stride == 1 || L.stride == 2, "conv: stride %d", L.stride);
  D3F_CHECK(!L.up0 || (L.Hv % 2 == 0 && L.Wv % 2 == 0), "conv: up-sampled extent must be even");
  D3F_CHECK(L.CinReal > 0 && L.CinReal <= L.C0 + L.C1, "conv: CinReal");

  const int B = L.B, K = L.KH;
  L.Cin = L.C0 + L.C1;
  L.Ho = (L.Hv + 2 * L.pad - K) / L.stride + 1;
  L.Wo = (L.Wv + 2 * L.pad - K) / L.stride + 1;
  L.CoutPad = (int)round_up(L.Cout, 16);
  L.Kpad = (int)round_up((long)K * K * L.Cin, bke);
  L.CoutD = (int)round_up(L.Cout, ve);
  L.KpadD = (int)round_up((long)K * K * L.CoutD, bke);
  L.CinRows = (int)round_up(L.Cin, 16);
  L.C0Rows = (int)round_up(L.C0, 16);
  L.C1Rows = (int)round_up(L.C1, 16);
  L.macs = (double)B * L.Ho * L.Wo * L.Cout * K * K * L.CinReal;
  static const bool no_upfold = prof_knob("D3F_NO_UPFOLD") != nullptr;
  L.upfold = !no_upfold && L.up0 && K == 3 && L.stride == 1 && L.pad == 1 && L.C0 % bke == 0 && L.C1 % bke == 0;
  L.parity = L.stride == 2 && L.C1 == 0 && L.CoutD % bke == 0 && ((K == 3 && L.pad == 1) || (K == 1 && L.pad == 0));
  L.wf = (size_t)L.CoutPad * L.Kpad * wsz;
  L.wd = (size_t)L.CinRows * L.KpadD * wsz;
  if (L.upfold) {
    L.wfc = (size_t)4 * L.CoutPad * (4 * L.C0 + 9 * L.C1) * wsz;
    L.wd4 = (size_t)L.C0Rows * 16 * L.CoutD * wsz;
    L.wds = (size_t)L.C1Rows * L.KpadD * wsz;
  }
  auto plan = [&](ConvParams& p, double flops) {
    p.plan_nets = L.plan_nets;
    p.flops = flops;
    const int rc = conv_igemm_plan(p, L.dtype, L.allow_splitk);
    L.splitk_floats = std::max(L.splitk_floats, conv_splitk_floats(p));
    return rc;
  };

  if (L.need_fwd) {
    ConvParams& f = L.fwd;
    f.B = B; f.Hv = L.Hv; f.Wv = L.Wv; f.C0 = L.C0; f.C1 = L.C1; f.cin_real = L.CinReal;
    f.H0s = L.Hv >> L.up0; f.W0s = L.Wv >> L.up0; f.shift0 = L.up0;
    f.Ho = L.Ho; f.Wo = L.Wo; f.Cout = L.Cout; f.CoutPad = L.CoutPad; f.Kpad = L.Kpad;
    f.KH = f.KW = K; f.stride = L.stride; f.pad = L.pad;
    f.M = B * L.Ho * L.Wo;
    f.mode = L.head ? CONV_HEAD_NCHW : CONV_RAW_STATS;
    if (L.upfold) {
      f.par = 3;
      f.shift0 = 0;
      f.Ho = f.H0s; f.Wo = f.W0s;
      f.M = B * f.H0s * f.W0s;
      f.Kpad = 4 * L.C0 + 9 * L.C1;
    }
    if (int rc = plan(f, 2.0 * L.macs)) return rc;
    L.wino = conv_winograd_applies(f, L.dtype);
    const bool fits = conv_winograd_fits(f, L.dtype);
    L.wino_rows = fits ? conv_winograd_stat_rows(f) : 0;
    L.wu = fits ? conv_winograd_filter_floats(f) * sizeof(float) : 0;
  }

  if (L.need_wgrad) {
    WgradParams g{};
    g.B = B; g.Hv = L.Hv; g.Wv = L.Wv; g.C0 = L.C0; g.C1 = L.C1;
    g.H0s = L.Hv >> L.up0; g.W0s = L.Wv >> L.up0; g.shift0 = L.up0;
    g.Ho = L.Ho; g.Wo = L.Wo; g.Cout = L.CoutD;
    g.KH = g.KW = K; g.stride = L.stride; g.pad = L.pad; g.M = B * L.Ho * L.Wo;
    g.cin_real = L.CinReal;
    g.flops = 2.0 * L.macs;
    g.plan_nets = L.plan_nets;
    if (int rc = wgrad_layer_plan(L.wl, g, L.sdtype)) return rc;
    L.wslab_bytes = wgrad_layer_partial_floats(L.wl) * sizeof(float);
  }

  if (!L.need_dgrad) return 0;
  D3F_CHECK(L.stride == 2 ? (L.Ho * 2 == L.Hv && L.Wo * 2 == L.Wv) : (L.Ho == L.Hv && L.Wo == L.Wv),
            "conv_backward_data: needs a 'same' (stride 1) or exactly halving (stride 2) conv");
  ConvParams dy{};
  dy.B = B; dy.C0 = L.CoutD;
  dy.mode = CONV_DGRAD;
  ConvParams& d = L.dgrad;
  if (L.upfold) {
    ConvParams& l = L.dgrad_lo;
    l = dy;
    l.Hv = l.H0s = L.Hv; l.Wv = l.W0s = L.Wv;
    l.Ho = L.Hv / 2; l.Wo = L.Wv / 2;
    l.Cout = l.out_c0 = L.C0; l.CoutPad = L.C0Rows; l.Kpad = 16 * L.CoutD;
    l.KH = l.KW = 4; l.stride = 2; l.pad = 1;
    l.M = B * l.Ho * l.Wo;
    if (int rc = plan(l, 2.0 * L.macs * L.C0 / L.Cin)) return rc;
    if (L.C1 == 0) return 0;
    d = dy;
    d.Hv = d.H0s = d.Ho = L.Hv; d.Wv = d.W0s = d.Wo = L.Wv;
    d.Cout = d.out_c0 = L.C1; d.CoutPad = L.C1Rows; d.Kpad = L.KpadD;
    d.KH = d.KW = 3; d.stride = 1; d.pad = 1;
    d.M = B * L.Hv * L.Wv;
    return plan(d, 2.0 * L.macs * L.C1 / L.Cin);
  }
  d = dy;
  d.Cout = L.Cin; d.CoutPad = L.CinRows; d.Kpad = L.KpadD;
  d.out_c0 = L.C1 > 0 ? L.C0 : L.Cin;
  if (L.parity) {
    d.par = K == 3 ? 1 : 2;
    d.Hv = d.Ho = d.H0s = L.Ho; d.Wv = d.Wo = d.W0s = L.Wo;
    d.KH = d.KW = K == 3 ? 2 : 1; d.stride = 1; d.pad = 0;
    d.M = B * L.Ho * L.Wo;
  } else {
    const int s2 = L.stride == 2 ? 1 : 0;
    d.Hv = L.Hv; d.Wv = L.Wv;
    d.H0s = L.Ho; d.W0s = L.Wo; d.shift0 = s2; d.zi = s2;
    d.Ho = L.Hv; d.Wo = L.Wv;
    d.KH = d.KW = K; d.stride = 1; d.pad = K - 1 - L.pad;
    d.M = B * L.Hv * L.Wv;
    d.sum2 = (L.want_sum2 && L.up0 && L.C1 == 0) ? 1 : 0;
  }
  return plan(d, 2.0 * L.macs);
}

static void net_conv(ConvParams& p, const NetSplit* ns) {
  if (ns != nullptr) {
    p.nets = ns->nets;
    p.net_ws = p.net_out0 = p.net_scale = ns->ws;
  }
}

int conv_layer_forward(const ConvLayer& L, const ConvFwdBufs& b, bool wino, hipStream_t s, const NetSplit* ns) {
  ConvParams p = L.fwd;
  p.src0 = b.src0; p.src1 = b.src1; p.w = b.w; p.out0 = b.out;
  net_conv(p, ns);
  if (L.head) {
    p.mode = CONV_HEAD_NCHW;
    p.scale = b.bias;
    if (ns != nullptr) {
      p.net_out0 = ns->out;
      p.net_scale = ns->par;
    }
    return conv_igemm_launch(p, L.dtype, s);
  }
  p.partial = p.splitk > 1 ? b.slabs : nullptr;
  if (b.scale != nullptr) {
    p.mode = CONV_EVAL_FUSED;
    p.scale = b.scale; p.shift = b.shift; p.res = b.res; p.relu = b.relu;
  } else {
    p.mode = CONV_RAW_STATS;
    p.stats = b.stats;
    if (wino) p.stat_rows = L.wino_rows;
  }
  return wino ? conv_winograd_launch(p, s) : conv_igemm_launch(p, L.dtype, s);
}

int conv_layer_dgrad(const ConvLayer& L, const ConvDgradBufs& b, hipStream_t s, const NetSplit* ns) {
  ConvParams p = L.upfold ? L.dgrad_lo : L.dgrad;
  p.src0 = b.dy; p.w = b.w; p.out0 = b.dx0; p.acc0 = b.acc0;
  if (!L.upfold) {
    p.out1 = b.dx1;
    p.acc1 = b.acc1;
  }
  p.partial = p.splitk > 1 ? b.slabs : nullptr;
  p.bn_y = b.bn_y; p.bn_coef = b.bn_coef; p.bn_partial = b.bn_partial; p.bn_a = b.bn_a;
  net_conv(p, ns);
  if (p.par == 2 && !p.acc0) {
    const NetSplit nv = net_split_or_single(ns);
    for (int n = 0; n < nv.nets; ++n)
      D3F_HIP(hipMemsetAsync(reinterpret_cast<char*>(b.dx0) + (size_t)n * nv.ws, 0,
                             (size_t)4 * p.M * p.Cout * (L.sdtype == D3F_F32 ? 4 : 2), s));
  }
  if (int rc = conv_igemm_launch(p, L.dtype, s)) return rc;
  if (!L.upfold || L.C1 == 0) return 0;
  ConvParams k = L.dgrad;
  k.src0 = b.dy; k.w = b.w_skip; k.out0 = b.dx1; k.acc0 = b.acc1;
  k.partial = k.splitk > 1 ? b.slabs : nullptr;
  net_conv(k, ns);
  return conv_igemm_launch(k, L.dtype, s);
}

int conv_pack_entry(const ConvLayer& L, long w_off, size_t wf_off, size_t wd_off, bool fwd, bool dgrad, uint32_t block0,
                    PackEntry& e) {
  const int taps = L.KH * L.KW;
  const long nf = fwd ? (long)L.CoutPad * L.Kpad : 0, nd = dgrad ? (long)L.CinRows * L.KpadD : 0;
  D3F_CHECK((!fwd || L.Kpad >= taps * L.Cin) && (!dgrad || L.KpadD >= taps * L.CoutD), "pack_weights: padded K too small");
  const int extent = std::max({L.Cout, L.CinReal, L.Cin, L.CoutPad, L.Kpad, L.CinRows, L.CoutD, L.KpadD});
  D3F_CHECK(extent < 65536 && nf + nd < 0x7fffffffL,
            "pack_weights: the layer exceeds the packing table (extents below 65536, fewer than 2^31 packed elements): "
            "extent %d, %ld elements", extent, nf + nd);
  D3F_CHECK(w_off >= 0 && w_off <= 0xffffffffL && wf_off % 16 == 0 && wd_off % 16 == 0 && (wf_off >> 4) < 0xffffffffull &&
                (wd_off >> 4) < 0xffffffffull,
            "pack_weights: layer out of table range");
  D3F_CHECK(taps <= PACK_LDS_ROW, "pack_weights: %d taps exceed the tile", taps);
  int CT = 32;
  while (CT * taps > PACK_LDS_ROW) CT >>= 1;
  const int crows = std::max(fwd ? L.Cin : 0, dgrad ? L.CinRows : 0);
  const int nrows = std::max(fwd ? L.CoutPad : 0, dgrad ? L.CoutD : 0);
  unsigned mul, shr;
  fast_div_setup((unsigned)taps, &mul, &shr);
  e = PackEntry{};
  e.w_off = (uint32_t)w_off;
  e.wf_off16 = (uint32_t)(wf_off >> 4);
  e.wd_off16 = (uint32_t)(wd_off >> 4);
  e.block0 = block0;
  e.Cout = (uint16_t)L.Cout; e.CinReal = (uint16_t)L.CinReal; e.Cin = (uint16_t)L.Cin;
  e.taps = (uint16_t)taps; e.CoutPad = (uint16_t)L.CoutPad; e.Kpad = (uint16_t)L.Kpad;
  e.CinRows = (uint16_t)L.CinRows; e.CoutD = (uint16_t)L.CoutD; e.KpadD = (uint16_t)L.KpadD;
  e.has_f = fwd ? 1 : 0;
  e.has_d = dgrad ? 1 : 0;
  e.conv_stride = (dgrad && L.parity) ? 2 : 1;
  e.CT = (uint16_t)CT;
  e.ctiles = (uint16_t)((crows + CT - 1) / CT);
  e.taps_mul = mul;
  e.taps_shr = (uint16_t)shr;
  e.ct_log2 = (uint16_t)__builtin_ctz((unsigned)CT);
  return e.ctiles * ((nrows + PACK_NT - 1) / PACK_NT);
}

}
```

### denoising_diffusion_deep_fake_amd/csrc/engine.h

```cpp
#pragma once
#include <string>
#include <vector>

#include "common.h"
#include "pointwise.h"

namespace d3f {

struct TensorD {
  size_t off = 0;
  int H = 0, W = 0, C = 0;
  long elems(int B) const { return (long)B * H * W * C; }
};

struct ParamInfo {
  std::string name;
  int shape[4];
  int ndim;
  long offset;
  long numel;
};

struct BnInfo {
  std::string prefix;
  int C;
  long rm_off, rv_off;
};

struct Unit : ConvLayer {
  std::string conv_name;
  int in0 = -1, in1 = -1, y = -1, a = -1;
  bool bn = true, bias = false;
  BnLayer norm;
  int res_tensor = -1, res_unit = -1;
  long w_off = -1, bias_off = -1, g_off = -1, b_off = -1, rm_off = -1, rv_off = -1;
  size_t wf_off = 0, wd_off = 0;
  size_t coef_off = 0;
  int segment = 0;
  size_t dy_off = 0;
  size_t wfc_off = 0, wd4_off = 0, wds_off = 0;
  size_t wu_off = 0;
  size_t wslab_off = 0;
};

enum BwdKind { BW_HEAD, BW_UNIT, BW_SUM2X2, BW_POOL };
struct BwdOp {
  BwdKind kind;
  int unit = -1;
  int dA = -1;
  int fuse_for_unit = -1;
  int fused_rows = 0;
  bool mask = true;
  int dres = -1;
  bool dres_acc = false;
  int dst0 = -1, dst1 = -1;
  bool acc0 = false, acc1 = false;
  bool dst0_is_full_scratch = false;
  int C = 0, Hl = 0, Wl = 0;
  int segment = 0;
};

struct NetIO {
  long params = 0, bnstats = 0, grads = 0, x = 0, out = 0, dout = 0;
};

class UnetEngine {
 public:
  ~UnetEngine();
  int build(const char* encoder, int in_channels, int classes, int B, int H, int W, int dtype, int nets = 1,
            int plan_nets = 1);

  int pack_weights(const float* params, void* ws, hipStream_t s, const NetIO* io = nullptr) const;
  int forward(const float* params, float* bnstats, const float* x, float* out, void* ws, int training,
              hipStream_t s, const NetIO* io = nullptr) const;
  int backward(const float* params, const float* dout, float* grads, void* ws, int seg_begin,
               int seg_end, hipStream_t s, int join = 1, const NetIO* io = nullptr) const;
  int backward_join(hipStream_t s) const;
  hipStream_t side_stream() const;
  int predict_u8(const float* params, float* bnstats, const uint8_t* bgr_in, uint8_t* bgr_out,
                 const float mean[3], const float stdv[3], void* ws, int use_graph, hipStream_t s) const;
  int predict_frames_u8(const float* params, float* bnstats, const uint8_t* raw_in, int src_h, int src_w, int x1, int y1,
                        int cw, int ch, uint8_t* pair_out, const float mean[3], const float stdv[3], void* ws,
                        int use_graph, hipStream_t s) const;
  int forward_graph(const float* params, float* bnstats, const float* x, float* out, void* ws, hipStream_t s) const;
  struct StepArgs {
    float* params; float* bnstats; float* grads; float* exp_avg; float* exp_avg_sq;
    const float* image; const float* noise; const float* y_uniform;
    float* noisy; float* pred; float* gpred; float* loss_out; float* loss_ws;
    const float* adam_coef;
    float lam, lo, hi;
  };
  int train_step(const StepArgs& a, void* ws, int use_graph, hipStream_t s) const;
  typedef int (*AllReduceFn)(void* ctx, float* data, int64_t count, void* stream);
  bool bn_sync_installed() const { return bn_sync_.fn != nullptr; }
  void set_bn_sync(AllReduceFn fn, void* ctx, int world) { bn_sync_ = BnSync{fn, ctx, world > 0 ? world : 1}; }
  int export_tensor(const char* name, const void* ws, float* out_nchw, hipStream_t s) const;
  int export_shape(const char* name, int32_t dims[3]) const;

  std::vector<ParamInfo> params;
  std::vector<BnInfo> bns;
  long param_floats = 0, bnstat_floats = 0;
  size_t workspace_bytes = 0;
  int num_segments = 4;
  long seg_grad_begin[8] = {0}, seg_grad_end[8] = {0};
  int B = 0, H = 0, W = 0, dtype = 0, in_channels = 3, classes = 3;
  int nets = 1, plan_nets = 1;
  size_t net_ws_stride = 0;
  int cdtype = 0;
  double fwd_flops = 0, bwd_flops = 0;
  std::vector<Unit> units;

 private:
  int esize() const { return dtype == D3F_F32 ? 4 : 2; }
  int wsize() const { return cdtype == D3F_F32X3 ? 6 : esize(); }
  int ve() const { return dtype == D3F_F32 ? 4 : 8; }
  const TensorD* find_export(const char* name) const;
  int new_tensor(int H_, int W_, int C_);
  int new_grad(int tensor_id);
  size_t alloc(size_t bytes);
  int add_unit(const std::string& conv_name, const std::string& bn_name, int in0, int in1, int up0,
               int Cout, int k, int stride, int pad, bool bn, bool bias, bool relu, bool apply,
               int segment);

  std::vector<TensorD> tensors;
  std::vector<TensorD> gtensors;
  std::vector<int> grad_of;
  std::vector<bool> grad_init;
  std::vector<BwdOp> bwd_ops;
  std::vector<int> fwd_order_;
  mutable hipStream_t side_ = nullptr;
  mutable std::vector<hipEvent_t> ev_dy_;
  mutable hipEvent_t ev_join_ = nullptr;
  mutable hipEvent_t ev_seg_ = nullptr;
  mutable bool side_dirty_ = false;
  int ensure_streams() const;
  mutable hipEvent_t ev_pack_in_ = nullptr, ev_pack_done_ = nullptr, ev_pack_mid_ = nullptr;
  mutable bool pack_pending_ = false, pack_mid_pending_ = false;
  int first_mid_unit_ = -1;
  int first_late_unit_ = -1;
  int forward_body(const float* params, float* bnstats, float* out, char* ws, int training, hipStream_t s,
                   const NetSplit* ns = nullptr) const;
  bool make_split(const NetIO* io, long in_delta, NetSplit* ns) const;
  int predict_u8_launches(const float* params, float* bnstats, const uint8_t* bgr_in, uint8_t* bgr_out,
                          const float mean255[3], const float std255[3], char* ws, hipStream_t s) const;
  int predict_frames_u8_launches(const float* params, float* bnstats, const uint8_t* raw_in, const int geo[6],
                                 uint8_t* pair_out, const float mean255[3], const float std255[3], char* ws,
                                 hipStream_t s) const;
  struct GraphKey {
    const void* ptr[5];
    float cst[6];
    int geo[6];
  };
  struct GraphSlot {
    hipGraphExec_t exec = nullptr;
    GraphKey key = {};
  };
  template <typename F>
  int graph_replay(GraphSlot& slot, const GraphKey& key, hipStream_t s, F&& launches) const;
  int wait_for_packed_weights(hipStream_t s) const;
  mutable hipStream_t gstream_ = nullptr;
  mutable GraphSlot g_predict_, g_eval_, g_frames_;
  BnSync bn_sync_{nullptr, nullptr, 1};
  const BnSync* bn_sync() const { return bn_sync_.fn != nullptr ? &bn_sync_ : nullptr; }
  int train_step_launches(const StepArgs& a, void* ws, hipStream_t s) const;
  mutable hipGraphExec_t g_step_ = nullptr;
  mutable StepArgs g_step_key_{};
  mutable const void* g_step_ws_ = nullptr;
  mutable hipEvent_t ev_gin_ = nullptr, ev_gout_ = nullptr;
  size_t head_nchw_off = 0;
  size_t ws_top = 0;
  int t_x = -1, t_pool = -1, head = -1, conv1 = -1;
  size_t pool_idx_off = 0, stats_off = 0, bnpart_off = 0, dz_off = 0, dfull_off = 0,
         bsum_off = 0, splitk_off = 0;
  size_t stats_bytes = 0, bnpart_bytes = 0, dy_bytes = 0, dz_bytes = 0, dfull_bytes = 0, splitk_bytes = 0;
};

int channel_sum_nchw_launch(const float* x, int B, int C, long HW, float* partial, float* out,
                            hipStream_t stream, const NetSplit* ns = nullptr);

}
```

### denoising_diffusion_deep_fake_amd/csrc/engine.hip

```cpp
#include "engine.h"
#include <vector>

#include <cstdio>
#include <cstdlib>
#include <cstring>

namespace d3f {

constexpr int CS_PP = 16;
__global__ __launch_bounds__(256) void channel_sum_partial_kernel(const float* __restrict__ x, int C, long HW,
                                                                  float* __restrict__ partial, int nb, long net_in,
                                                                  long net_ws) {
  __shared__ float red[256];
  const int seg = blockIdx.x, c = blockIdx.y, b = (int)blockIdx.z % nb;
  if ((int)blockIdx.z >= nb) {
    net_shift(x, net_in); net_shift(partial, net_ws);
  }
  const float* __restrict__ plane = x + ((long)b * C + c) * HW;
  const long per = (HW + CS_PP - 1) / CS_PP, lo = (long)seg * per, hi = lo + per < HW ? lo + per : HW;
  float s = 0.f;
  if ((HW & 3) == 0 && (per & 3) == 0) {
    for (long i = lo + 4 * threadIdx.x; i < hi; i += 4 * 256) {
      const float4 v = *reinterpret_cast<const float4*>(plane + i);
      s += (v.x + v.y) + (v.z + v.w);
// ... 245 lines not shown
    op.segment = u.segment;
    if (u.need_dgrad) {
      if (u.upfold) {
        op.dst0 = grad_dst(u.in0, &op.acc0);
        if (u.in1 >= 0) op.dst1 = grad_dst(u.in1, &op.acc1);
        D3F_CHECK(u.segment == 0, "plan: unit %s: a folded up-sampling layer outside the decoder bucket", u.conv_name.c_str());
      } else if (u.up0 && !u.dgrad.sum2) {
        op.dst0_is_full_scratch = true;
        if (u.in1 >= 0) op.dst1 = grad_dst(u.in1, &op.acc1);
      } else {
        op.dst0 = grad_dst(u.in0, &op.acc0);
      }
    }
    bwd_ops.push_back(op);
    if (u.need_dgrad && u.up0 && !u.upfold && !u.dgrad.sum2) {
      BwdOp s;
      s.kind = BW_SUM2X2; s.unit = ui; s.C = u.C0; s.Hl = u.Hv / 2; s.Wl = u.Wv / 2; s.segment = u.segment;
      bool acc;
      s.dst0 = grad_dst(u.in0, &acc);
      D3F_CHECK(!acc, "plan: up-sampled tensor has two consumers");
      bwd_ops.push_back(s);
    }
    return 0;
  };
  {
    BwdOp h;
    h.kind = BW_HEAD; h.unit = head; h.segment = 0;
    h.dst0 = grad_dst(units[head].in0, &h.acc0);
    bwd_ops.push_back(h);
  }
  for (int i = 4; i >= 0; --i) {
    const DBlk& d = dec_blocks[i];
    if (int rc = emit_unit(d.u2, grad_of[units[d.u2].a], true, -1, false)) return rc;
    if (int rc = emit_unit(d.u1, grad_of[units[d.u1].a], true, -1, false)) return rc;
  }
  for (int bi = (int)enc_blocks.size() - 1; bi >= 0; --bi) {
    const Blk& b = enc_blocks[bi];
    const Unit& u2 = units[b.u2];
    D3F_CHECK(grad_of[u2.a] >= 0, "plan: block output without gradient");
    int dres;
    bool dres_acc = false;
    if (b.ud >= 0) dres = -2;
    else dres = grad_dst(u2.res_tensor, &dres_acc);
    if (int rc = emit_unit(b.u2, grad_of[u2.a], true, dres, dres_acc)) return rc;
    if (int rc = emit_unit(b.u1, grad_of[units[b.u1].a], true, -1, false)) return rc;
    if (b.ud >= 0)
      if (int rc = emit_unit(b.ud, -2, false, -1, false)) return rc;
  }
  {
    BwdOp p;
    p.kind = BW_POOL; p.segment = 3;
    p.dA = grad_of[t_pool];
    D3F_CHECK(p.dA >= 0, "plan: pool output without gradient");
    p.dst0 = grad_dst(f1, &p.acc0);
    bwd_ops.push_back(p);
  }
  if (int rc = emit_unit(conv1, grad_of[f1], true, -1, false)) return rc;

  static const bool no_fused_reduce = getenv("D3F_NO_FUSED_BN_REDUCE") != nullptr;
  if (!no_fused_reduce) {
    auto writes = [&](const BwdOp& o, int gid) {
      if (o.kind == BW_UNIT || o.kind == BW_HEAD) {
        if (units[o.unit].need_dgrad && !o.dst0_is_full_scratch && o.dst0 == gid) return true;
        if (o.dst1 == gid) return true;
        if (o.kind == BW_UNIT && o.dres == gid) return true;
      }
      return (o.kind == BW_SUM2X2 || o.kind == BW_POOL) && o.dst0 == gid;
    };
    for (size_t j = 0; j + 1 < bwd_ops.size(); ++j) {
      BwdOp& pj = bwd_ops[j];
      if (!(pj.kind == BW_UNIT || pj.kind == BW_HEAD)) continue;
      const Unit& up = units[pj.unit];
      const ConvParams& pd = up.upfold ? up.dgrad_lo : up.dgrad;
      if (!up.need_dgrad || pd.par || pj.dst0_is_full_scratch || (pj.dst1 >= 0 && !up.upfold) || pj.dst0 < 0) continue;
      BwdOp& ck = bwd_ops[j + 1];
      if (ck.kind != BW_UNIT || ck.dA != pj.dst0) continue;
      bool last = true;
      for (size_t k = j + 1; k < bwd_ops.size(); ++k) last = last && !writes(bwd_ops[k], pj.dst0);
      const Unit& uc = units[ck.unit];
      if (!last || !(uc.bn && ck.mask)) continue;
      D3F_CHECK(pd.Cout == uc.Cout && pd.M == (pd.sum2 ? 4 : 1) * B * uc.Ho * uc.Wo && pd.out_c0 == pd.Cout,
                "plan: fused BatchNorm reduce shape mismatch (%s -> %s)", up.conv_name.c_str(), uc.conv_name.c_str());
      pj.fuse_for_unit = ck.unit;
      ck.fused_rows = pd.splitk > 1 ? pd.stat_rows : pd.tiles_m;
    }
  }

  for (const BwdOp& op : bwd_ops) {
    if (op.kind != BW_UNIT) continue;
    Unit& u = units[op.unit];
    u.norm.res = u.res_tensor >= 0 ? BN_RES_TENSOR : u.res_unit >= 0 ? BN_RES_LAYER : BN_RES_NONE;
    u.norm.mask = !op.mask ? BN_MASK_NONE : u.norm.res == BN_RES_NONE ? BN_MASK_FROM_Y : BN_MASK_FROM_A;
    u.norm.fused_rows = op.fused_rows;
  }
  for (Unit& u : units) {
    if (!u.bn) continue;
    bn_layer_plan(u.norm);
    stats_bytes = std::max(stats_bytes, u.norm.stat_floats * sizeof(float));
    bnpart_bytes = std::max(bnpart_bytes, u.norm.part_floats * sizeof(float));
  }

  stats_off = alloc(stats_bytes);
  bnpart_off = alloc(bnpart_bytes);
  dz_off = alloc(dz_bytes);
  dfull_off = alloc(dfull_bytes);
  bsum_off = alloc(channel_sum_partial_floats(B, classes) * sizeof(float));
  splitk_off = alloc(splitk_bytes);
  head_nchw_off = alloc((size_t)B * classes * H * W * sizeof(float));
  net_ws_stride = nets > 1 ? (size_t)round_up((long)ws_top, 4096) : 0;
  workspace_bytes = nets > 1 ? net_ws_stride * nets : ws_top;

  long layer3_start = -1, layer4_start = -1, dec_start = -1;
  for (const auto& p : params) {
    if (layer3_start < 0 && p.name.rfind("encoder.layer3.", 0) == 0) layer3_start = p.offset;
    if (layer4_start < 0 && p.name.rfind("encoder.layer4.", 0) == 0) layer4_start = p.offset;
    if (dec_start < 0 && p.name.rfind("decoder.", 0) == 0) dec_start = p.offset;
  }
  num_segments = 4;
  seg_grad_begin[0] = dec_start;     seg_grad_end[0] = param_floats;
  seg_grad_begin[1] = layer4_start;  seg_grad_end[1] = dec_start;
  seg_grad_begin[2] = layer3_start;  seg_grad_end[2] = layer4_start;
  seg_grad_begin[3] = 0;             seg_grad_end[3] = layer3_start;
  fwd_order_.clear();
  fwd_order_.push_back(conv1);
  fwd_order_.push_back(-1);
  for (const auto& b : enc_blocks) {
    fwd_order_.push_back(b.u1);
    if (b.ud >= 0) fwd_order_.push_back(b.ud);
    fwd_order_.push_back(b.u2);
  }
  for (const auto& d : dec_blocks) {
    fwd_order_.push_back(d.u1);
    fwd_order_.push_back(d.u2);
  }
  fwd_order_.push_back(head);
  return 0;
}

static int shared_side_stream(hipStream_t* out) {
  constexpr int MAXDEV = 64;
  static hipStream_t streams[MAXDEV] = {};
  int dev = 0;
  D3F_HIP(hipGetDevice(&dev));
  D3F_CHECK(dev >= 0 && dev < MAXDEV, "side stream: device index %d", dev);
  if (streams[dev] == nullptr) {
    int least = 0, greatest = 0;
    D3F_HIP(hipDeviceGetStreamPriorityRange(&least, &greatest));
    D3F_HIP(hipStreamCreateWithPriority(&streams[dev], hipStreamNonBlocking, least));
  }
  *out = streams[dev];
  return 0;
}

int UnetEngine::ensure_streams() const {
  if (side_ != nullptr) return 0;
  if (int rc = shared_side_stream(&side_)) return rc;
  D3F_HIP(hipEventCreateWithFlags(&ev_join_, hipEventDisableTiming));
  D3F_HIP(hipEventCreateWithFlags(&ev_seg_, hipEventDisableTiming));
  D3F_HIP(hipEventCreateWithFlags(&ev_pack_in_, hipEventDisableTiming));
  D3F_HIP(hipEventCreateWithFlags(&ev_pack_done_, hipEventDisableTiming));
  D3F_HIP(hipEventCreateWithFlags(&ev_pack_mid_, hipEventDisableTiming));
  return 0;
}

bool UnetEngine::make_split(const NetIO* io, long in_delta, NetSplit* ns) const {
  if (nets <= 1) return false;
  ns->nets = nets;
  ns->ws = (long)net_ws_stride;
  ns->par = io->params;
  ns->grad = io->grads;
  ns->bn = io->bnstats;
  ns->in = in_delta;
  ns->out = io->out;
  return true;
}

int UnetEngine::pack_weights(const float* params0_, void* ws0_, hipStream_t s, const NetIO* io) const {
  D3F_CHECK((int)units.size() <= PACK_MAX_LAYERS, "pack_weights: %d layers exceed the table", (int)units.size());
  D3F_CHECK(nets == 1 || io != nullptr, "pack_weights: a pair engine needs the second network's offsets");
  static const bool sync_pack = getenv("D3F_NO_ASYNC_PACK") != nullptr;
  const bool async = !sync_pack && first_late_unit_ > 0;
  const int mid = async ? first_mid_unit_ : -1;
  auto params_of = [&](int n) { return reinterpret_cast<const float*>(reinterpret_cast<const char*>(params0_) + (n ? io->params : 0)); };
  auto ws_of = [&](int n) { return reinterpret_cast<char*>(ws0_) + (size_t)n * net_ws_stride; };
  auto part_of = [&](int ui) { return ui >= first_late_unit_ ? 2 : (mid > 0 && ui >= mid) ? 1 : 0; };
  for (int part = 0; part < 3; ++part) {
    if (part == 1 && mid <= 0) continue;
    PackTable t;
    t.n = 0;
    uint32_t blocks = 0;
    for (int ui = 0; ui < (int)units.size(); ++ui) {
      const Unit& u = units[ui];
      if (first_late_unit_ > 0 && part_of(ui) != part) continue;
      if (first_late_unit_ <= 0 && part != 0) continue;
      if (u.upfold) continue;
      const int nb = conv_pack_entry(u, u.w_off, u.wf_off, u.wd_off, true, u.need_dgrad, blocks, t.e[t.n++]);
      if (nb < 0) return nb;
      blocks += (uint32_t)nb;
    }
    hipStream_t ps = s;
    if (part >= 1 && async) {
      if (int rc = ensure_streams()) return rc;
      if (part == 1 || mid <= 0) {
        D3F_HIP(hipEventRecord(ev_pack_in_, s));
        D3F_HIP(hipStreamWaitEvent(side_, ev_pack_in_, 0));
      }
      ps = side_;
    }
    for (int n = 0; n < nets; ++n) {
      const float* params_ = params_of(n);
      char* ws = ws_of(n);
      if (t.n > 0)
        if (int rc = pack_all_launch(cdtype, params_, ws, t, (int)blocks, ps)) return rc;
      for (int ui = 0; ui < (int)units.size(); ++ui) {
        const Unit& u = units[ui];
        if (!u.wino) continue;
        if (first_late_unit_ > 0 ? part_of(ui) != part : part != 0) continue;
        if (int rc = conv_winograd_pack_launch(params_ + u.w_off, reinterpret_cast<float*>(ws + u.wu_off), u.Cout, u.Cin, ps))
          return rc;
      }
    }
    if (part == 1 && async) {
      D3F_HIP(hipEventRecord(ev_pack_mid_, side_));
      pack_mid_pending_ = true;
    }
    if (part == 2 || (first_late_unit_ <= 0 && part == 0)) {
      for (int n = 0; n < nets; ++n) {
        const float* params_ = params_of(n);
        char* ws = ws_of(n);
        for (const Unit& u : units)
          if (u.upfold)
            if (int rc = pack_up_launch(cdtype, params_ + u.w_off, u.Cout, u.C0, u.C1, ws + u.wfc_off, u.CoutPad,
                                        u.need_dgrad ? ws + u.wd4_off : nullptr, u.C0Rows,
                                        (u.need_dgrad && u.C1 > 0) ? ws + u.wds_off : nullptr, u.C1Rows, ps))
              return rc;
      }
    }
    if (part == 2 && async) {
      D3F_HIP(hipEventRecord(ev_pack_done_, side_));
      pack_pending_ = true;
    }
  }
  return 0;
}

int UnetEngine::forward(const float* params_, float* bnstats, const float* x, float* out, void* ws_,
                        int training, hipStream_t s, const NetIO* io) const {
  char* ws = reinterpret_cast<char*>(ws_);
  D3F_CHECK(nets == 1 || (io != nullptr && training), "unet: the pair engine runs train-mode passes and needs the second "
            "network's offsets");
  NetSplit split{};
  const NetSplit* ns = make_split(io, io ? io->x : 0, &split) ? &split : nullptr;
  if (int rc = nchw_to_nhwc_launch(dtype, x, ws + tensors[t_x].off, B, in_channels, H, W, tensors[t_x].C, s, ns))
    return rc;
  return forward_body(params_, bnstats, out, ws, training, s, ns);
}

int UnetEngine::forward_body(const float* params_, float* bnstats, float* out, char* ws, int training,
                             hipStream_t s, const NetSplit* ns) const {
  auto T = [&](int tid) { return ws + tensors[tid].off; };
  auto coef = [&](const Unit& u) { return reinterpret_cast<float*>(ws + u.coef_off); };
  D3F_CHECK(ns == nullptr || (training && bn_sync() == nullptr), "unet: the pair engine runs train-mode passes with "
            "per-GPU BatchNorm statistics");
  if (!training) {
    BnEvalTable t;
    t.n = 0;
    for (const Unit& u : units)
      if (u.bn) {
        D3F_CHECK(t.n < PACK_MAX_LAYERS && u.coef_off % 16 == 0, "eval coefficients: table overflow");
        BnEvalEntry& e = t.e[t.n++];
        e.g_off = (uint32_t)u.g_off; e.b_off = (uint32_t)u.b_off;
        e.rm_off = (uint32_t)u.rm_off; e.rv_off = (uint32_t)u.rv_off;
        e.coef_off16 = (uint32_t)(u.coef_off >> 4);
        e.C = u.Cout;
      }
    if (int rc = bn_eval_coeff_all_launch(params_, bnstats, ws, t, s)) return rc;
  }
  for (int ui : fwd_order_) {
    if (ui < 0) {
      const TensorD& f1 = tensors[units[conv1].a];
      if (int rc = maxpool3x3s2_fwd_launch(dtype, T(units[conv1].a), T(t_pool),
                                           reinterpret_cast<uint8_t*>(ws + pool_idx_off), B, f1.H, f1.W,
                                           f1.C, s, ns))
        return rc;
      continue;
    }
    const Unit& u = units[ui];
    if (pack_mid_pending_ && ui >= first_mid_unit_) {
      D3F_HIP(hipStreamWaitEvent(s, ev_pack_mid_, 0));
      pack_mid_pending_ = false;
    }
    if (pack_pending_ && ui >= first_late_unit_) {
      D3F_HIP(hipStreamWaitEvent(s, ev_pack_done_, 0));
      pack_pending_ = false;
    }
    ConvFwdBufs b;
    b.src0 = T(u.in0);
    b.src1 = u.in1 >= 0 ? T(u.in1) : nullptr;
    b.w = ws + (u.wino ? u.wu_off : u.upfold ? u.wfc_off : u.wf_off);
    b.slabs = reinterpret_cast<float*>(ws + splitk_off);
    if (!u.bn) {
      b.out = out;
      b.bias = params_ + u.bias_off;
      if (int rc = conv_layer_forward(u, b, false, s, ns)) return rc;
      continue;
    }
    const Unit* ds = u.res_unit >= 0 ? &units[u.res_unit] : nullptr;
    if (training) {
      b.out = T(u.y);
      b.stats = reinterpret_cast<float*>(ws + stats_off);
      if (int rc = conv_layer_forward(u, b, u.wino, s, ns)) return rc;
      BnBufs n;
      n.stats = b.stats;
      n.gamma = params_ + u.g_off; n.beta = params_ + u.b_off;
      n.running_mean = bnstats + u.rm_off; n.running_var = bnstats + u.rv_off;
      n.coef = coef(u);
      n.y = T(u.y); n.a = u.a >= 0 ? T(u.a) : nullptr;
      n.res = u.res_tensor >= 0 ? T(u.res_tensor) : (ds ? T(ds->y) : nullptr);
      n.res_coef = ds ? coef(*ds) : nullptr;
      if (int rc = bn_layer_forward(u.norm, n, bn_sync(), s, ns)) return rc;
    } else {
      b.scale = bn_coef(coef(u), u.Cout, BN_SCALE);
      b.shift = bn_coef(coef(u), u.Cout, BN_SHIFT);
      b.relu = u.norm.relu ? 1 : 0;
      if (u.norm.apply) {
        b.out = T(u.a);
        b.res = u.res_tensor >= 0 ? T(u.res_tensor) : (ds ? T(ds->y) : nullptr);
      } else {
        b.out = T(u.y);
      }
      if (int rc = conv_layer_forward(u, b, u.wino, s, ns)) return rc;
    }
  }
  return 0;
}

int UnetEngine::predict_u8_launches(const float* params_, float* bnstats, const uint8_t* bgr_in, uint8_t* bgr_out,
                                    const float mean255[3], const float std255[3], char* ws, hipStream_t s) const {
  if (int rc = u8bgr_to_nhwc_launch(dtype, bgr_in, ws + tensors[t_x].off, (long)B * H * W, tensors[t_x].C, mean255,
                                    std255, s))
    return rc;
  float* head_out = reinterpret_cast<float*>(ws + head_nchw_off);
  if (int rc = forward_body(params_, bnstats, head_out, ws, 0, s)) return rc;
  return nchw_to_u8bgr_launch(head_out, bgr_out, B, H, W, 3L * W, mean255, std255, s);
}

int UnetEngine::predict_u8(const float* params_, float* bnstats, const uint8_t* bgr_in, uint8_t* bgr_out,
                           const float mean[3], const float stdv[3], void* ws_, int use_graph,
                           hipStream_t s) const {
  D3F_CHECK(in_channels == 3 && classes == 3, "predict_u8: 3-channel frames only (in %d, out %d)", in_channels, classes);
  char* ws = reinterpret_cast<char*>(ws_);
  float m255[3], s255[3];
  for (int c = 0; c < 3; ++c) {
    m255[c] = mean[c] * 255.0f;
    s255[c] = stdv[c] * 255.0f;
  }
  if (!use_graph) return predict_u8_launches(params_, bnstats, bgr_in, bgr_out, m255, s255, ws, s);
  const GraphKey key = {{params_, bnstats, bgr_in, bgr_out, ws_}, {m255[0], m255[1], m255[2], s255[0], s255[1], s255[2]}, {}};
  return graph_replay(g_predict_, key, s, [&](hipStream_t gs) {
    return predict_u8_launches(params_, bnstats, bgr_in, bgr_out, m255, s255, ws, gs);
  });
}

int UnetEngine::predict_frames_u8_launches(const float* params_, float* bnstats, const uint8_t* raw_in, const int geo[6],
                                           uint8_t* pair_out, const float mean255[3], const float std255[3], char* ws,
                                           hipStream_t s) const {
  if (int rc = crop_resize_cubic_u8_nhwc_launch(dtype, raw_in, B, geo[0], geo[1], geo[2], geo[3], geo[4], geo[5], pair_out,
                                                H, W, 6L * W, ws + tensors[t_x].off, tensors[t_x].C, mean255, std255, s))
    return rc;
  float* head_out = reinterpret_cast<float*>(ws + head_nchw_off);
  if (int rc = forward_body(params_, bnstats, head_out, ws, 0, s)) return rc;
  return nchw_to_u8bgr_launch(head_out, pair_out + 3L * W, B, H, W, 6L * W, mean255, std255, s);
}

int UnetEngine::predict_frames_u8(const float* params_, float* bnstats, const uint8_t* raw_in, int src_h, int src_w, int x1,
                                  int y1, int cw, int ch, uint8_t* pair_out, const float mean[3], const float stdv[3],
                                  void* ws_, int use_graph, hipStream_t s) const {
  D3F_CHECK(in_channels == 3 && classes == 3, "predict_frames_u8: 3-channel frames only (in %d, out %d)", in_channels,
            classes);
  char* ws = reinterpret_cast<char*>(ws_);
  float m255[3], s255[3];
  for (int c = 0; c < 3; ++c) {
    m255[c] = mean[c] * 255.0f;
    s255[c] = stdv[c] * 255.0f;
  }
  if (int rc = crop_resize_cubic_check(B, src_h, src_w, x1, y1, cw, ch, H, W, 6L * W)) return rc;
  const int geo[6] = {src_h, src_w, x1, y1, cw, ch};
  if (!use_graph) return predict_frames_u8_launches(params_, bnstats, raw_in, geo, pair_out, m255, s255, ws, s);
  const GraphKey key = {{params_, bnstats, raw_in, pair_out, ws_},
                        {m255[0], m255[1], m255[2], s255[0], s255[1], s255[2]},
                        {src_h, src_w, x1, y1, cw, ch}};
  return graph_replay(g_frames_, key, s, [&](hipStream_t gs) {
    return predict_frames_u8_launches(params_, bnstats, raw_in, geo, pair_out, m255, s255, ws, gs);
  });
}

int UnetEngine::forward_graph(const float* params_, float* bnstats, const float* x, float* out, void* ws_,
                              hipStream_t s) const {
  const GraphKey key = {{params_, bnstats, x, out, ws_}, {}, {}};
  return graph_replay(g_eval_, key, s, [&](hipStream_t gs) { return forward(params_, bnstats, x, out, ws_, 0, gs); });
}

int UnetEngine::train_step_launches(const StepArgs& a, void* ws_, hipStream_t s) const {
  const long per_image = (long)in_channels * H * W;
  if (int rc = pack_weights(a.params, ws_, s)) return rc;
  if (int rc = noise_blend_launch(a.image, a.noise, a.y_uniform, a.lam, a.noisy, nullptr, B, per_image, s)) return rc;
  if (int rc = forward(a.params, a.bnstats, a.noisy, a.pred, ws_, 1, s)) return rc;
  if (int rc = mse_ssim_loss_launch(a.pred, a.image, a.lo, a.hi, a.loss_out, a.gpred, a.loss_ws, B, H, W, s)) return rc;
  if (int rc = backward(a.params, a.gpred, a.grads, ws_, 0, num_segments, s, 1)) return rc;
  return adam_step_dev_launch(a.params, a.grads, a.exp_avg, a.exp_avg_sq, param_floats, a.adam_coef, s);
}

int UnetEngine::train_step(const StepArgs& a, void* ws_, int use_graph, hipStream_t s) const {
  D3F_CHECK(in_channels == 3 && classes == 3, "train_step: the (MSE + 1 - SSIM) / 2 objective is defined on 3-channel images");
  if (!use_graph) return train_step_launches(a, ws_, s);
  if (int rc = wait_for_packed_weights(s)) return rc;
  if (int rc = ensure_streams()) return rc;
  if (gstream_ == nullptr) {
    D3F_HIP(hipStreamCreateWithFlags(&gstream_, hipStreamNonBlocking));
    D3F_HIP(hipEventCreateWithFlags(&ev_gin_, hipEventDisableTiming));
    D3F_HIP(hipEventCreateWithFlags(&ev_gout_, hipEventDisableTiming));
  }
  const bool same = g_step_ != nullptr && g_step_ws_ == ws_ && memcmp(&a, &g_step_key_, sizeof(StepArgs)) == 0;
  if (!same) {
    if (g_step_) {
      (void)hipGraphExecDestroy(g_step_);
      g_step_ = nullptr;
    }
    hipGraph_t graph = nullptr;
    D3F_HIP(hipStreamBeginCapture(gstream_, hipStreamCaptureModeThreadLocal));
    const int rc = train_step_launches(a, ws_, gstream_);
    const hipError_t e = hipStreamEndCapture(gstream_, &graph);
    pack_pending_ = pack_mid_pending_ = false;
    side_dirty_ = false;
    if (rc != 0) {
      if (graph) (void)hipGraphDestroy(graph);
      return rc;
    }
    D3F_HIP(e);
    const hipError_t ei = hipGraphInstantiate(&g_step_, graph, nullptr, nullptr, 0);
    (void)hipGraphDestroy(graph);
    D3F_HIP(ei);
    g_step_key_ = a;
    g_step_ws_ = ws_;
  }
  D3F_HIP(hipGraphLaunch(g_step_, s));
  return 0;
}

int UnetEngine::wait_for_packed_weights(hipStream_t s) const {
  if (pack_mid_pending_) {
    D3F_HIP(hipStreamWaitEvent(s, ev_pack_mid_, 0));
    pack_mid_pending_ = false;
  }
  if (pack_pending_) {
    D3F_HIP(hipStreamWaitEvent(s, ev_pack_done_, 0));
    pack_pending_ = false;
  }
  return 0;
}

template <typename F>
int UnetEngine::graph_replay(GraphSlot& slot, const GraphKey& key, hipStream_t s, F&& launches) const {
  if (int rc = wait_for_packed_weights(s)) return rc;
  if (gstream_ == nullptr) {
    D3F_HIP(hipStreamCreateWithFlags(&gstream_, hipStreamNonBlocking));
    D3F_HIP(hipEventCreateWithFlags(&ev_gin_, hipEventDisableTiming));
    D3F_HIP(hipEventCreateWithFlags(&ev_gout_, hipEventDisableTiming));
  }
  static_assert(sizeof(GraphKey) == 5 * sizeof(void*) + 6 * sizeof(float) + 6 * sizeof(int), "GraphKey is compared bytewise");
  const bool same = slot.exec != nullptr && memcmp(&key, &slot.key, sizeof(GraphKey)) == 0;
  if (!same) {
    if (slot.exec) {
      (void)hipGraphExecDestroy(slot.exec);
      slot.exec = nullptr;
    }
    hipGraph_t graph = nullptr;
    D3F_HIP(hipStreamBeginCapture(gstream_, hipStreamCaptureModeThreadLocal));
    const int rc = launches(gstream_);
    const hipError_t e = hipStreamEndCapture(gstream_, &graph);
    if (rc != 0) {
      if (graph) (void)hipGraphDestroy(graph);
      return rc;
    }
    D3F_HIP(e);
    const hipError_t ei = hipGraphInstantiate(&slot.exec, graph, nullptr, nullptr, 0);
    (void)hipGraphDestroy(graph);
    D3F_HIP(ei);
    slot.key = key;
  }
  D3F_HIP(hipEventRecord(ev_gin_, s));
  D3F_HIP(hipStreamWaitEvent(gstream_, ev_gin_, 0));
  D3F_HIP(hipGraphLaunch(slot.exec, gstream_));
  D3F_HIP(hipEventRecord(ev_gout_, gstream_));
  D3F_HIP(hipStreamWaitEvent(s, ev_gout_, 0));
  return 0;
}

UnetEngine::~UnetEngine() {
  if (g_predict_.exec) (void)hipGraphExecDestroy(g_predict_.exec);
  if (g_eval_.exec) (void)hipGraphExecDestroy(g_eval_.exec);
  if (g_frames_.exec) (void)hipGraphExecDestroy(g_frames_.exec);
  if (g_step_) (void)hipGraphExecDestroy(g_step_);
  if (ev_gin_) (void)hipEventDestroy(ev_gin_);
  if (ev_gout_) (void)hipEventDestroy(ev_gout_);
  if (gstream_) (void)hipStreamDestroy(gstream_);
  for (hipEvent_t e : ev_dy_)
    if (e) (void)hipEventDestroy(e);
  if (ev_join_) (void)hipEventDestroy(ev_join_);
  if (ev_seg_) (void)hipEventDestroy(ev_seg_);
  if (ev_pack_in_) (void)hipEventDestroy(ev_pack_in_);
  if (ev_pack_done_) (void)hipEventDestroy(ev_pack_done_);
  if (ev_pack_mid_) (void)hipEventDestroy(ev_pack_mid_);
}

static bool serial_backward() {
  static const bool serial = getenv("D3F_SERIAL_BACKWARD") != nullptr;
  return serial;
}

hipStream_t UnetEngine::side_stream() const {
  if (serial_backward() || ensure_streams() != 0) return nullptr;
  return side_;
}

int UnetEngine::backward_join(hipStream_t s) const {
  if (side_ != nullptr && side_dirty_) {
    D3F_HIP(hipEventRecord(ev_join_, side_));
    D3F_HIP(hipStreamWaitEvent(s, ev_join_, 0));
    side_dirty_ = false;
  }
  return 0;
}

int UnetEngine::backward(const float* params_, const float* dout, float* grads, void* ws_,
                         int seg_begin, int seg_end, hipStream_t s, int join, const NetIO* io) const {
  char* ws = reinterpret_cast<char*>(ws_);
  D3F_CHECK(nets == 1 || (io != nullptr && bn_sync() == nullptr), "unet: the pair engine needs the second network's "
            "offsets and runs with per-GPU BatchNorm statistics");
  NetSplit split{};
  const NetSplit* ns = make_split(io, io ? io->dout : 0, &split) ? &split : nullptr;
  auto T = [&](int tid) { return ws + tensors[tid].off; };
  auto G = [&](int gid) { return gid == -2 ? ws + dz_off : ws + gtensors[gid].off; };
  auto coef = [&](const Unit& u) { return reinterpret_cast<float*>(ws + u.coef_off); };
  const bool serial = serial_backward();
#ifdef D3F_PROFILING
  static const char* abl = getenv("D3F_ABLATE_BACKWARD");
  const bool skip_w = abl && strchr(abl, 'w'), skip_d = abl && strchr(abl, 'd'), skip_b = abl && strchr(abl, 'b');
  const bool skip_r = abl && strchr(abl, 'r');
#else
  constexpr bool skip_w = false, skip_d = false, skip_b = false, skip_r = false;
#endif
  if (!serial)
    if (int rc = ensure_streams()) return rc;
  hipStream_t ws_stream = serial ? s : side_;
  size_t next_event = 0;
  bool side_used = false;
  constexpr int defer = 3;
  std::vector<int> pending;
  int pending_segment = -1;
  bool head_bias_pending = false;
  auto flush_pending = [&]() -> int {
    if (pending.empty()) return 0;
    if (!serial) {
      if (next_event == ev_dy_.size()) {
        hipEvent_t e = nullptr;
        D3F_HIP(hipEventCreateWithFlags(&e, hipEventDisableTiming));
        ev_dy_.push_back(e);
      }
      D3F_HIP(hipEventRecord(ev_dy_[next_event], s));
      D3F_HIP(hipStreamWaitEvent(side_, ev_dy_[next_event], 0));
      ++next_event;
      side_used = true;
    }
    if (head_bias_pending) {
      const Unit& uh = units[head];
      if (int rc = channel_sum_nchw_launch(dout, B, uh.Cout, (long)uh.Ho * uh.Wo, reinterpret_cast<float*>(ws + bsum_off),
                                           grads + uh.bias_off, ws_stream, ns))
        return rc;
      head_bias_pending = false;
    }
    for (int ui : pending) {
      const Unit& u = units[ui];
      WgradReduceBatch red;
      if (int rc = wgrad_layer_launch_deferred(u.wl, ws + u.dy_off, T(u.in0), u.in1 >= 0 ? T(u.in1) : nullptr,
                                               reinterpret_cast<float*>(ws + u.wslab_off), grads + u.w_off, u.Cout,
                                               u.CinReal, cdtype, red, ws_stream, ns))
        return rc;
      if (!skip_r)
        if (int rc = wgrad_reduce_batch_launch(red, ws_stream)) return rc;
    }
    pending.clear();
    return 0;
  };
  for (const BwdOp& op : bwd_ops) {
    if (op.segment < seg_begin || op.segment >= seg_end) continue;
    if (op.segment != pending_segment) {
      if (int rc = flush_pending()) return rc;
      pending_segment = op.segment;
    }
    if (op.kind == BW_SUM2X2) {
      if (int rc = sum2x2_launch(dtype, ws + dfull_off, G(op.dst0), B, op.Hl, op.Wl, op.C, s, ns)) return rc;
      continue;
    }
    if (op.kind == BW_POOL) {
      const TensorD& f1 = tensors[units[conv1].a];
      if (int rc = maxpool3x3s2_bwd_launch(dtype, G(op.dA), reinterpret_cast<uint8_t*>(ws + pool_idx_off),
                                           G(op.dst0), op.acc0 ? 1 : 0, B, f1.H, f1.W, f1.C, s, ns))
        return rc;
      continue;
    }
    const Unit& u = units[op.unit];
    char* dy = ws + u.dy_off;
    if (op.kind == BW_HEAD) {
      if (int rc = nchw_to_nhwc_launch(dtype, dout, dy, B, u.Cout, u.Ho, u.Wo, u.CoutD, s, ns)) return rc;
      if (skip_w) {
        if (int rc = channel_sum_nchw_launch(dout, B, u.Cout, (long)u.Ho * u.Wo,
                                             reinterpret_cast<float*>(ws + bsum_off), grads + u.bias_off, s, ns))
          return rc;
      } else {
        head_bias_pending = true;
      }
    } else if (!skip_b) {
      BnBufs n;
      n.stats = reinterpret_cast<float*>(ws + bnpart_off);
      n.gamma = params_ + u.g_off;
      n.coef = coef(u);
      n.y = T(u.y); n.a = u.a >= 0 ? T(u.a) : nullptr;
      n.dA = G(op.dA); n.dy = dy;
      n.dres = op.dres == -1 ? nullptr : G(op.dres); n.dres_acc = op.dres_acc ? 1 : 0;
      n.dgamma = grads + u.g_off; n.dbeta = grads + u.b_off;
      if (int rc = bn_layer_backward(u.norm, n, bn_sync(), s, ns)) return rc;
    }
    if (!skip_w) {
      pending.push_back(op.unit);
      if ((int)pending.size() >= defer)
        if (int rc = flush_pending()) return rc;
    }
    if (u.need_dgrad && !skip_d) {
      ConvDgradBufs d;
      d.dy = dy;
      d.w = ws + (u.upfold ? u.wd4_off : u.wd_off);
      d.w_skip = ws + u.wds_off;
      if (op.dst0_is_full_scratch) {
        d.dx0 = ws + dfull_off;
      } else {
        d.dx0 = G(op.dst0);
        d.acc0 = op.acc0 ? 1 : 0;
      }
      d.dx1 = op.dst1 >= 0 ? G(op.dst1) : nullptr;
      d.acc1 = op.acc1 ? 1 : 0;
      d.slabs = reinterpret_cast<float*>(ws + splitk_off);
      if (op.fuse_for_unit >= 0) {
        const Unit& uc = units[op.fuse_for_unit];
        d.bn_y = T(uc.y);
        d.bn_coef = bn_coef(coef(uc), uc.Cout, BN_MEAN);
        d.bn_partial = reinterpret_cast<float*>(ws + bnpart_off);
        d.bn_a = uc.norm.mask == BN_MASK_FROM_A ? T(uc.a) : nullptr;
      }
      if (int rc = conv_layer_dgrad(u, d, s, ns)) return rc;
    }
  }
  if (int rc = flush_pending()) return rc;
  if (!serial && side_used) side_dirty_ = true;
  if (!serial && !join) {
    D3F_HIP(hipEventRecord(ev_seg_, s));
    D3F_HIP(hipStreamWaitEvent(side_, ev_seg_, 0));
    side_dirty_ = true;
  } else if (!serial) {
    if (int rc = backward_join(s)) return rc;
  }
  return 0;
}

const TensorD* UnetEngine::find_export(const char* name) const {
  const std::string n(name);
  const size_t colon = n.rfind(':');
  if (colon == std::string::npos) return nullptr;
  const std::string un = n.substr(0, colon), kind = n.substr(colon + 1);
  if (kind != "y" && kind != "a" && kind != "da") return nullptr;
  for (const Unit& u : units) {
    if (u.conv_name != un) continue;
    const int tid = kind == "y" ? u.y : u.a;
    if (tid < 0) return nullptr;
    if (kind == "da") return grad_of[tid] >= 0 ? &gtensors[grad_of[tid]] : nullptr;
    return &tensors[tid];
  }
  return nullptr;
}

int UnetEngine::export_tensor(const char* name, const void* ws_, float* out_nchw, hipStream_t s) const {
  const TensorD* t = find_export(name);
  D3F_CHECK(t != nullptr, "export: no tensor named '%s' (expected '<conv name>:y|a|da')", name);
  return nhwc_to_nchw_launch(dtype, reinterpret_cast<const char*>(ws_) + t->off, out_nchw, B, t->C, t->H, t->W, t->C, s);
}

int UnetEngine::export_shape(const char* name, int32_t dims[3]) const {
  const TensorD* t = find_export(name);
  D3F_CHECK(t != nullptr, "export: no tensor named '%s' (expected '<conv name>:y|a|da')", name);
  dims[0] = t->C; dims[1] = t->H; dims[2] = t->W;
  return 0;
}

}
```

### denoising_diffusion_deep_fake_amd/ops.py

```python
import ctypes as C

import torch

from . import _lib
from ._lib import ConvDesc, check, ptr, stream_ptr

F32, BF16, F32X3 = _lib.F32, _lib.BF16, _lib.F32X3


def _tdtype(dtype):
    return torch.bfloat16 if dtype == BF16 else torch.float32


def _dev(t):
    if t.device.type != "cuda":
        raise _lib.D3FError("libd3f_hip ops need tensors on the HIP device (no CPU fallback)")
    return t.device


def make_desc(B, H, W, C0, C1, Cout, k, stride, pad, upsample0=False, cin_real=None):
    return ConvDesc(B, H, W, C0, C1, 1 if upsample0 else 0, Cout, k, k, stride, pad,
                    cin_real if cin_real is not None else C0 + C1)


def out_hw(d):
    return (d.H + 2 * d.pad - d.KH) // d.stride + 1, (d.W + 2 * d.pad - d.KW) // d.stride + 1


def nchw_to_nhwc(x, cpad, dtype=F32):
    B, Cc, H, W = x.shape
    out = torch.empty((B, H, W, cpad), dtype=_tdtype(dtype), device=_dev(x))
    check(_lib.lib().d3f_nchw_to_nhwc(dtype, ptr(x.contiguous().float()), ptr(out), B, Cc, H, W, cpad, stream_ptr()))
    return out


def nhwc_to_nchw(x, c, dtype=F32):
    B, H, W, cpad = x.shape
    out = torch.empty((B, c, H, W), dtype=torch.float32, device=_dev(x))
    check(_lib.lib().d3f_nhwc_to_nchw(dtype, ptr(x.contiguous()), ptr(out), B, c, H, W, cpad, stream_ptr()))
    return out


def pack_weights(d, w, dtype=F32, dgrad=True):
    L = _lib.lib()
    dev = _dev(w)
    wf = torch.empty(L.d3f_conv_packed_bytes(dtype, C.byref(d), 0), dtype=torch.uint8, device=dev)
    wd = torch.empty(L.d3f_conv_packed_bytes(dtype, C.byref(d), 1), dtype=torch.uint8, device=dev) if dgrad else None
    check(L.d3f_conv_pack_weights(dtype, C.byref(d), ptr(w.contiguous().float()), ptr(wf), ptr(wd), stream_ptr()))
    return wf, wd


def _conv_ws(d, dtype, which, dev, splitk):
    if not splitk:
        return None
    n = _lib.lib().d3f_conv_workspace_bytes(dtype, C.byref(d), which)
    return torch.empty(max(n, 16), dtype=torch.uint8, device=dev)


def conv_forward(d, src0, src1, wf, dtype=F32, want_stats=True, splitk=False):
    L = _lib.lib()
    ho, wo = out_hw(d)
    y = torch.empty((d.B, ho, wo, d.Cout), dtype=_tdtype(dtype), device=_dev(src0))
    ws = _conv_ws(d, dtype, 0, y.device, splitk)
    tiles = C.c_int()
    n = L.d3f_conv_stats_floats(dtype, C.byref(d), int(splitk), C.byref(tiles))
    stats = torch.zeros(n, dtype=torch.float32, device=y.device) if want_stats else None
    check(L.d3f_conv_forward(dtype, C.byref(d), ptr(src0), ptr(src1), ptr(wf), ptr(y), ptr(stats), ptr(ws),
                             stream_ptr()))
    return y, stats, tiles.value


def conv_winograd_applies(d, dtype=F32):
    return bool(_lib.lib().d3f_conv_winograd_applies(dtype, C.byref(d)))


def conv_winograd_pack(d, w):
    L = _lib.lib()
    n = L.d3f_conv_winograd_filter_bytes(C.byref(d))
    if n == 0:
        raise _lib.D3FError("conv_winograd_pack: the layer does not fit the Winograd kernel")
    u = torch.empty(n, dtype=torch.uint8, device=_dev(w))
    check(L.d3f_conv_winograd_pack(C.byref(d), ptr(w.contiguous().float()), ptr(u), stream_ptr()))
    return u


def conv_winograd_forward(d, src0, u, want_stats=True, scale=None, shift=None, residual=None, relu=False):
    L = _lib.lib()
    y = torch.empty((d.B, d.H, d.W, d.Cout), dtype=torch.float32, device=_dev(src0))
    tiles = C.c_int()
    n = L.d3f_conv_winograd_stats_floats(C.byref(d), C.byref(tiles))
    stats = torch.zeros(n, dtype=torch.float32, device=y.device) if (want_stats and scale is None) else None
    check(L.d3f_conv_winograd_forward(C.byref(d), ptr(src0), ptr(u), ptr(y), ptr(stats), ptr(scale), ptr(shift),
                                      ptr(residual), int(relu), stream_ptr()))
    return y, stats, tiles.value


def conv_upsample_folded(d, dtype=F32):
    return bool(d.upsample0) and bool(_lib.lib().d3f_conv_upsample_folded(dtype, C.byref(d)))


def conv_backward_data(d, dy, wd, dtype=F32, dx0=None, dx1=None, acc0=False, acc1=False, splitk=False, summed=None):
    dev = _dev(dy)
    ws = _conv_ws(d, dtype, 1, dev, splitk)
    folded = bool(d.upsample0) and bool(_lib.lib().d3f_conv_upsample_folded(dtype, C.byref(d)))
    if bool(d.upsample0) and not folded and summed is not False and \
            bool(_lib.lib().d3f_conv_upsample_summed(dtype, C.byref(d))):
        d = ConvDesc(*[getattr(d, n) for n, _ in ConvDesc._fields_])
        d.upsample0 = 2
        folded = True
    low = (d.B, d.H // 2, d.W // 2, d.C0)
    if d.upsample0 and not folded:
        if acc0 or dx0 is not None:
            raise ValueError("conv_backward_data: an up-sampled source that is not folded takes no dx0 / acc0")
        full = torch.empty((d.B, d.H, d.W, d.C0), dtype=_tdtype(dtype), device=dev)
    elif dx0 is None:
        full = None
        dx0 = torch.empty(low if d.upsample0 else (d.B, d.H, d.W, d.C0), dtype=_tdtype(dtype), device=dev)
    else:
        full = None
    if dx1 is None and d.C1 > 0:
        dx1 = torch.empty((d.B, d.H, d.W, d.C1), dtype=_tdtype(dtype), device=dev)
    check(_lib.lib().d3f_conv_backward_data(dtype, C.byref(d), ptr(dy), ptr(wd), ptr(full if full is not None else dx0),
                                            ptr(dx1), int(acc0), int(acc1), ptr(ws), stream_ptr()))
    if full is not None:
        dx0 = upsample2x_backward(full, dtype)
    return dx0, dx1


def conv_backward_weight(d, dy, src0, src1, dtype=F32):
    L = _lib.lib()
    ws = torch.empty(L.d3f_conv_backward_weight_workspace_bytes(dtype, C.byref(d)), dtype=torch.uint8, device=_dev(dy))
    dw = torch.empty((d.Cout, d.CinReal, d.KH, d.KW), dtype=torch.float32, device=dy.device)
    check(L.d3f_conv_backward_weight(dtype, C.byref(d), ptr(dy), ptr(src0), ptr(src1), ptr(ws), ptr(dw), stream_ptr()))
    return dw


def bn_finalize(stats, tiles, Cc, count, gamma, beta, running_mean=None, running_var=None):
    coef = torch.empty(4 * Cc, dtype=torch.float32, device=_dev(stats))
    check(_lib.lib().d3f_bn_finalize(ptr(stats), tiles, Cc, count, ptr(gamma), ptr(beta), ptr(running_mean),
                                     ptr(running_var), ptr(coef), stream_ptr()))
    return coef


def bn_apply(y, coef, residual=None, relu=True, dtype=F32):
    Cc = y.shape[-1]
    out = torch.empty_like(y)
    check(_lib.lib().d3f_bn_apply(dtype, ptr(y), ptr(coef), Cc, y.numel() // Cc, ptr(residual), int(relu),
                                  ptr(out), stream_ptr()))
    return out


def bn_backward(dA, a, y, coef, gamma, want_dres=False, dtype=F32):
    L = _lib.lib()
    Cc = y.shape[-1]
    rows = y.numel() // Cc
    ws = torch.empty(L.d3f_bn_backward_workspace_bytes(dtype, Cc, rows), dtype=torch.uint8, device=_dev(y))
    dy = torch.empty_like(y)
    dres = torch.empty_like(y) if want_dres else None
    dgamma = torch.empty(Cc, dtype=torch.float32, device=y.device)
    dbeta = torch.empty(Cc, dtype=torch.float32, device=y.device)
    check(L.d3f_bn_backward(dtype, ptr(dA), ptr(a), ptr(y), ptr(coef), ptr(gamma), Cc, rows, ptr(dy), ptr(dres),
                            ptr(dgamma), ptr(dbeta), ptr(ws), stream_ptr()))
    return dy, dres, dgamma, dbeta


def bn_desc(C_, rows, dtype=F32, cpad=None, apply=True, relu=True, res=0, mask=0, fwd_rows=0, fused_rows=0,
            allow_fused=True, plan_nets=1):
    return _lib.BnDesc(dtype, C_, C_ if cpad is None else cpad, rows, int(apply), int(relu), res, mask, fwd_rows,
                       fused_rows, int(allow_fused), plan_nets)


def bn_layer_plan(d):
    p = _lib.BnPlan()
    check(_lib.lib().d3f_bn_layer_plan(C.byref(d), C.byref(p)))
    return p


def bn_layer_forward(d, stats, gamma, beta, coef, y, a=None, res=None, res_coef=None, running_mean=None,
                     running_var=None):
    check(_lib.lib().d3f_bn_layer_forward(C.byref(d), ptr(stats), ptr(gamma), ptr(beta), ptr(running_mean),
                                          ptr(running_var), ptr(coef), ptr(y), ptr(res), ptr(res_coef), ptr(a),
                                          stream_ptr()))


def bn_layer_backward(d, partial, gamma, coef, y, dA, dy, a=None, dres=None, dres_acc=False, dgamma=None, dbeta=None):
    check(_lib.lib().d3f_bn_layer_backward(C.byref(d), ptr(partial), ptr(gamma), ptr(coef), ptr(y), ptr(a), ptr(dA),
                                           ptr(dy), ptr(dres), int(dres_acc), ptr(dgamma), ptr(dbeta), stream_ptr()))


def maxpool_forward(x, dtype=F32):
    B, H, W, Cc = x.shape
    out = torch.empty((B, H // 2, W // 2, Cc), dtype=x.dtype, device=_dev(x))
    idx = torch.empty((B, H // 2, W // 2, Cc), dtype=torch.uint8, device=x.device)
    check(_lib.lib().d3f_maxpool3x3s2_forward(dtype, ptr(x), ptr(out), ptr(idx), B, H, W, Cc, stream_ptr()))
    return out, idx


def maxpool_backward(dout, idx, H, W, dtype=F32, din=None):
    B, _, _, Cc = dout.shape
    acc = din is not None
    if din is None:
        din = torch.empty((B, H, W, Cc), dtype=dout.dtype, device=_dev(dout))
    check(_lib.lib().d3f_maxpool3x3s2_backward(dtype, ptr(dout), ptr(idx), ptr(din), int(acc), B, H, W, Cc, stream_ptr()))
    return din


def upsample2x_backward(dfull, dtype=F32):
    B, H, W, Cc = dfull.shape
    out = torch.empty((B, H // 2, W // 2, Cc), dtype=dfull.dtype, device=_dev(dfull))
    check(_lib.lib().d3f_upsample2x_backward(dtype, ptr(dfull), ptr(out), B, H // 2, W // 2, Cc, stream_ptr()))
    return out


def affine_warp(x, theta):
    x = x.contiguous().float()
    B, Cc, H, W = x.shape
    theta = theta.to(device=_dev(x), dtype=torch.float32).contiguous()
    if theta.shape != (B, 2, 3):
        raise ValueError(f"theta must be [{B}, 2, 3], got {list(theta.shape)}")
    out = torch.empty_like(x)
    check(_lib.lib().d3f_affine_warp(ptr(x), ptr(theta), ptr(out), B, Cc, H, W, stream_ptr()))
    return out
# ... 172 lines not shown
```

### include/d3f_hip.h

```cpp
#ifndef D3F_HIP_H
#define D3F_HIP_H
#include <stddef.h>
#include <stdint.h>

#ifdef __cplusplus
extern "C" {
#endif

#define D3F_F32 0
#define D3F_BF16 1
#define D3F_F32X3 2

int d3f_version(void);
const char* d3f_last_error(void);
const char* d3f_source_digest(void);

int d3f_profile_enable(int max_launches);
int d3f_profile_classes(int mask);
int d3f_profile_collect(double ms[3], int64_t launches[3], double flops[3]);

typedef struct d3f_unet* d3f_unet_t;

int d3f_unet_create(const char* encoder_name, int in_channels, int classes, int B, int H, int W,
                    int dtype, d3f_unet_t* out);
int d3f_unet_destroy(d3f_unet_t h);

int d3f_unet_create_nets(const char* encoder_name, int in_channels, int classes, int B, int H, int W, int dtype,
                         int nets, int plan_nets, d3f_unet_t* out);
int d3f_unet_nets(d3f_unet_t h);
size_t d3f_unet_net_workspace_stride(d3f_unet_t h);
int d3f_unet_pair_pack_weights(d3f_unet_t h, const float* const params[2], void* workspace, void* stream);
int d3f_unet_pair_forward(d3f_unet_t h, const float* const params[2], float* const bnstats[2], const float* const x[2],
                          float* const out[2], void* workspace, void* stream);
int d3f_unet_pair_backward(d3f_unet_t h, const float* const params[2], const float* const grad_out[2],
                           float* const grads[2], void* workspace, int seg_begin, int seg_end, int join, void* stream);

int d3f_unet_num_params(d3f_unet_t h);
int d3f_unet_param_info(d3f_unet_t h, int i, char* name, int name_cap, int32_t shape[4], int* ndim,
                        int64_t* offset);
int64_t d3f_unet_param_floats(d3f_unet_t h);
int d3f_unet_num_bn(d3f_unet_t h);
int d3f_unet_bn_info(d3f_unet_t h, int i, char* prefix, int prefix_cap, int* C, int64_t* rm_offset,
                     int64_t* rv_offset);
int64_t d3f_unet_bnstat_floats(d3f_unet_t h);
size_t d3f_unet_workspace_bytes(d3f_unet_t h);
double d3f_unet_forward_flops(d3f_unet_t h);
double d3f_unet_backward_flops(d3f_unet_t h);

int d3f_unet_pack_weights(d3f_unet_t h, const float* params, void* workspace, void* stream);
int d3f_unet_forward(d3f_unet_t h, const float* params, float* bnstats, const float* x, float* out,
                     void* workspace, int training, void* stream);
int d3f_unet_forward_graph(d3f_unet_t h, const float* params, float* bnstats, const float* x, float* out,
                           void* workspace, void* stream);
int d3f_unet_predict_u8(d3f_unet_t h, const float* params, float* bnstats, const uint8_t* bgr_in, uint8_t* bgr_out,
                        const float mean[3], const float std[3], void* workspace, int use_graph, void* stream);
int d3f_unet_predict_frames_u8(d3f_unet_t h, const float* params, float* bnstats, const uint8_t* raw_in, int src_h,
                               int src_w, int x1, int y1, int cw, int ch, uint8_t* pair_out, const float mean[3],
                               const float std[3], void* workspace, int use_graph, void* stream);
int d3f_unet_num_segments(d3f_unet_t h);
int d3f_unet_plan_counts(d3f_unet_t h, int32_t fwd[16], int32_t dgrad[16], int32_t wgrad[16]);
int d3f_unet_segment_range(d3f_unet_t h, int segment, int64_t* begin, int64_t* end);
int d3f_unet_backward(d3f_unet_t h, const float* params, const float* grad_out, float* grads,
                      void* workspace, int seg_begin, int seg_end, void* stream);
int d3f_unet_backward_nojoin(d3f_unet_t h, const float* params, const float* grad_out, float* grads,
                             void* workspace, int seg_begin, int seg_end, void* stream);
int d3f_unet_side_stream(d3f_unet_t h, void** stream_out);
int d3f_unet_backward_join(d3f_unet_t h, void* stream);
typedef struct d3f_step_buffers {
  float* params; float* bnstats; float* grads; float* exp_avg; float* exp_avg_sq;
  const float* image;
  const float* noise;
  const float* y_uniform;
  float* noisy;
  float* pred;
  float* grad_pred;
  float* loss_out;
  void* loss_workspace;
  const float* adam_coef;
} d3f_step_buffers;
int d3f_adam_coefficients(float lr, float beta1, float beta2, float eps, int step, float grad_scale, float coef[8]);
int d3f_unet_train_step(d3f_unet_t h, const d3f_step_buffers* buffers, float lambda, float input_min, float input_max,
                        void* workspace, int use_graph, void* stream);
typedef int (*d3f_allreduce_fn)(void* ctx, float* data, int64_t count, void* stream);
int d3f_unet_set_bn_sync(d3f_unet_t h, d3f_allreduce_fn fn, void* ctx, int world_size);
int d3f_unet_export(d3f_unet_t h, const char* name, const void* workspace, float* out_nchw, void* stream);
int d3f_unet_export_shape(d3f_unet_t h, const char* name, int32_t dims[3]);

typedef struct d3f_conv_desc {
  int32_t B, H, W;
  int32_t C0, C1;
  int32_t upsample0;
  int32_t Cout, KH, KW, stride, pad;
  int32_t CinReal;
} d3f_conv_desc;

size_t d3f_conv_packed_bytes(int dtype, const d3f_conv_desc* d, int which);
int d3f_conv_pack_weights(int dtype, const d3f_conv_desc* d, const float* w, void* w_fwd, void* w_dgrad,
                          void* stream);
size_t d3f_conv_workspace_bytes(int dtype, const d3f_conv_desc* d, int which);
size_t d3f_conv_stats_floats(int dtype, const d3f_conv_desc* d, int with_workspace, int* tiles);
int d3f_conv_forward(int dtype, const d3f_conv_desc* d, const void* src0, const void* src1,
                     const void* w_fwd, void* y, float* stats, void* workspace, void* stream);
int d3f_conv_winograd_applies(int dtype, const d3f_conv_desc* d);
size_t d3f_conv_winograd_filter_bytes(const d3f_conv_desc* d);
size_t d3f_conv_winograd_stats_floats(const d3f_conv_desc* d, int* tiles);
int d3f_conv_winograd_pack(const d3f_conv_desc* d, const float* w, void* u, void* stream);
int d3f_conv_winograd_forward(const d3f_conv_desc* d, const void* src0, const void* u, void* y, float* stats,
                              const float* scale, const float* shift, const void* residual, int relu, void* stream);
int d3f_conv_upsample_folded(int dtype, const d3f_conv_desc* d);
int d3f_conv_upsample_summed(int dtype, const d3f_conv_desc* d);
int d3f_conv_backward_data(int dtype, const d3f_conv_desc* d, const void* dy, const void* w_dgrad,
                           void* dx0, void* dx1, int acc0, int acc1, void* workspace, void* stream);
size_t d3f_conv_backward_weight_workspace_bytes(int dtype, const d3f_conv_desc* d);
int d3f_conv_backward_weight(int dtype, const d3f_conv_desc* d, const void* dy, const void* src0,
                             const void* src1, void* workspace, float* dw, void* stream);

int d3f_bn_finalize(const float* stats, int tiles, int C, int64_t count, const float* gamma,
                    const float* beta, float* running_mean, float* running_var, float* coef, void* stream);
int d3f_bn_apply(int dtype, const void* y, const float* coef, int C, int64_t rows, const void* residual,
                 int relu, void* out, void* stream);
size_t d3f_bn_backward_workspace_bytes(int dtype, int C, int64_t rows);
int d3f_bn_backward(int dtype, const void* dA, const void* a_or_null, const void* y, const float* coef,
                    const float* gamma, int C, int64_t rows, void* dy, void* dres, float* dgamma,
                    float* dbeta, void* workspace, void* stream);

typedef struct d3f_bn_desc {
  int32_t dtype, C, Cpad;
  int64_t rows;
  int32_t apply, relu;
  int32_t res;
  int32_t mask;
  int32_t fwd_rows;
  int32_t fused_rows;
  int32_t allow_fused, plan_nets;
} d3f_bn_desc;
typedef struct d3f_bn_plan {
  int32_t fwd_fused, bwd_fused;
  int32_t reduce_blocks;
  int32_t bwd_rows;
  int64_t rows_per_block;
  uint64_t stat_floats;
  uint64_t part_floats;
} d3f_bn_plan;
#define D3F_BN_COEF_ROWS 7
int d3f_bn_layer_plan(const d3f_bn_desc* d, d3f_bn_plan* plan);
int d3f_bn_layer_forward(const d3f_bn_desc* d, float* stats, const float* gamma, const float* beta, float* running_mean,
                         float* running_var, float* coef, const void* y, const void* res, const float* res_coef, void* a,
                         void* stream);
int d3f_bn_layer_backward(const d3f_bn_desc* d, float* partial, const float* gamma, float* coef, const void* y,
                          const void* a, const void* dA, void* dy, void* dres, int dres_acc, float* dgamma, float* dbeta,
                          void* stream);
int d3f_unet_bn_layer(d3f_unet_t h, int i, d3f_bn_desc* d, d3f_bn_plan* plan);

int d3f_maxpool3x3s2_forward(int dtype, const void* in, void* out, uint8_t* idx, int B, int H, int W, int C, void* stream);
int d3f_maxpool3x3s2_backward(int dtype, const void* dout, const uint8_t* idx, void* din, int accumulate,
                              int B, int H, int W, int C, void* stream);
int d3f_upsample2x_backward(int dtype, const void* dfull, void* dlow, int B, int Hlow, int Wlow, int C, void* stream);
int d3f_nchw_to_nhwc(int dtype, const float* in, void* out, int B, int C, int H, int W, int Cpad, void* stream);
int d3f_nhwc_to_nchw(int dtype, const void* in, float* out, int B, int C, int H, int W, int Cpad, void* stream);
int d3f_u8rgb_normalise(const uint8_t* in_hwc, float* out_nchw, int B, int H, int W, const float mean[3],
                        const float std[3], void* stream);

int d3f_crop_resize_cubic_u8(const uint8_t* src, int B, int src_h, int src_w, int x1, int y1, int cw, int ch, uint8_t* dst,
                             int H, int W, int64_t dst_row_stride_bytes, void* stream);

int d3f_affine_warp(const float* in, const float* theta, float* out, int B, int C, int H, int W, void* stream);

int d3f_philox4x32_10(const uint32_t counter[4], const uint32_t key[2], uint32_t out[4]);

int d3f_affine_warp_rng(const float* in, float* out, uint64_t seed, uint64_t offset, int kind,
                        const float params[5], int B, int C, int H, int W, void* stream);
int d3f_affine_theta_draw(uint64_t seed, uint64_t offset, int kind, const float params[5],
                          float* theta, uint8_t* apply, int B, int H, int W, void* stream);

int d3f_noise_blend(const float* x, const float* noise, const float* y_uniform, float lam, float* out,
                    float* r_out_or_null, int B, int64_t per_image, void* stream);
int d3f_noise_blend_fixed(const float* x, const float* noise, const float* r, float* out, int B, int64_t per_image,
                          void* stream);
int d3f_noise_blend_rng(const float* x, uint64_t seed, uint64_t offset, float lam, float* out,
                        float* r_out_or_null, int B, int64_t per_image, void* stream);
int d3f_noise_blend_fixed_rng(const float* x, uint64_t seed, uint64_t offset, const float* r, float* out, int B,
                              int64_t per_image, void* stream);
int d3f_noise_draw(uint64_t seed, uint64_t offset, float* noise_or_null, float* y_or_null, int B, int64_t per_image,
                   void* stream);
size_t d3f_l1_per_image_workspace_bytes(int B);
int d3f_l1_per_image(const float* prediction, const float* target, float* out, void* workspace, int B,
                     int64_t per_image, void* stream);
size_t d3f_mse_ssim_loss_workspace_bytes(int B, int H, int W);
int d3f_mse_ssim_loss(const float* pred, const float* target, float input_min, float input_max,
                      float* loss_out, float* grad_pred, void* workspace, int B, int H, int W, void* stream);
int d3f_adam_step(float* params, const float* grads, float* exp_avg, float* exp_avg_sq, int64_t n,
                  float lr, float beta1, float beta2, float eps, int step, float grad_scale, void* stream);
int d3f_ema_lerp(float* ema, const float* online, int64_t n, float weight, void* stream);

#ifdef __cplusplus
}
#endif
#endif
```

Measured before the change: 2035 images/sec.

## Read NCHW input and master weights directly in stem conv and head dgrad

```diff
diff --git a/denoising_diffusion_deep_fake_amd/_lib.py b/denoising_diffusion_deep_fake_amd/_lib.py
--- a/denoising_diffusion_deep_fake_amd/_lib.py
+++ b/denoising_diffusion_deep_fake_amd/_lib.py
@@ -97,6 +97,8 @@
     "d3f_conv_winograd_pack": (_i, [_desc, _p, _p, _p]),
     "d3f_conv_winograd_forward": (_i, [_desc, _p, _p, _p, _p, _p, _p, _p, _i, _p]),
     "d3f_conv_backward_data": (_i, [_i, _desc, _p, _p, _p, _p, _i, _i, _p, _p]),
+    "d3f_conv_stem_forward": (_i, [_desc, _p, _i, _p, _i, _p, _p, _p]),
+    "d3f_conv_head_backward_data_nchw": (_i, [_desc, _p, _p, _p, _p]),
     "d3f_conv_backward_weight_workspace_bytes": (_sz, [_i, _desc]),
     "d3f_conv_backward_weight": (_i, [_i, _desc, _p, _p, _p, _p, _p, _p]),
     "d3f_bn_finalize": (_i, [_p, _i, _i, _i64, _p, _p, _p, _p, _p, _p]),
diff --git a/denoising_diffusion_deep_fake_amd/csrc/c_api.hip b/denoising_diffusion_deep_fake_amd/csrc/c_api.hip
--- a/denoising_diffusion_deep_fake_amd/csrc/c_api.hip
+++ b/denoising_diffusion_deep_fake_amd/csrc/c_api.hip
@@ -390,6 +390,21 @@
   b.slabs = reinterpret_cast<float*>(workspace);
   return conv_layer_forward(L, b, false, (hipStream_t)stream);
 }
+int d3f_conv_stem_forward(const d3f_conv_desc* d, const void* src0, int src_is_nchw, const void* w, int w_is_param, void* y,
+                          float* stats, void* stream) {
+  ConvLayer L;
+  if (int rc = plan(L, D3F_F32, d, PLAN_FWD)) return rc;
+  D3F_CHECK(conv_stem_reads_in_place(L),
+            "conv_stem_forward: needs the 7x7 / stride 2 / pad 3 layer of 3 channels padded to 4 that runs on the fp32 patch "
+            "kernel (output height a multiple of 8, width a multiple of 32, filters a multiple of 32)");
+  if (d->B == 0) return 0;
+  D3F_CHECK(src0 && w && y, "conv_stem_forward: null argument");
+  ConvFwdBufs b;
+  b.src0 = src0; b.w = w; b.out = y; b.stats = stats;
+  if (src_is_nchw) b.src_nchw = reinterpret_cast<const float*>(src0);
+  if (w_is_param) b.w_param = reinterpret_cast<const float*>(w);
+  return conv_layer_forward(L, b, false, (hipStream_t)stream);
+}
 static int wino_plan(ConvLayer& L, const d3f_conv_desc* d) {
   if (int rc = plan(L, D3F_F32, d, PLAN_FWD)) return rc;
   D3F_CHECK(L.wu != 0,
@@ -446,6 +461,19 @@
   b.dy = dy; b.w = w_dgrad; b.dx0 = dx0; b.dx1 = dx1; b.acc0 = acc0; b.acc1 = acc1;
   b.w_skip = L.upfold ? reinterpret_cast<const char*>(w_dgrad) + L.wd4 : nullptr;
   b.slabs = reinterpret_cast<float*>(workspace);
+  return conv_layer_dgrad(L, b, (hipStream_t)stream);
+}
+int d3f_conv_head_backward_data_nchw(const d3f_conv_desc* d, const float* dy_nchw, const void* w_dgrad, void* dx0,
+                                     void* stream) {
+  ConvLayer L;
+  if (int rc = plan(L, D3F_F32, d, PLAN_DGRAD)) return rc;
+  D3F_CHECK(conv_head_dgrad_reads_nchw(L),
+            "conv_head_backward_data_nchw: needs the 3x3 / stride 1 / pad 1 layer of 3 filters whose data gradient runs on "
+            "the fp32 patch kernel (16 channels, height a multiple of 4, width a multiple of 64)");
+  if (d->B == 0) return 0;
+  D3F_CHECK(dy_nchw && w_dgrad && dx0, "conv_head_backward_data_nchw: null argument");
+  ConvDgradBufs b;
+  b.dy = dy_nchw; b.dy_nchw = dy_nchw; b.w = w_dgrad; b.dx0 = dx0;
   return conv_layer_dgrad(L, b, (hipStream_t)stream);
 }
 size_t d3f_conv_backward_weight_workspace_bytes(int dtype, const d3f_conv_desc* d) {
diff --git a/denoising_diffusion_deep_fake_amd/csrc/common.h b/denoising_diffusion_deep_fake_amd/csrc/common.h
--- a/denoising_diffusion_deep_fake_amd/csrc/common.h
+++ b/denoising_diffusion_deep_fake_amd/csrc/common.h
@@ -79,6 +79,9 @@
 __device__ __forceinline__ uint4 buf_load16(__amdgpu_buffer_rsrc_t r, unsigned byte_off) {
   const u32x4_t v = __builtin_amdgcn_raw_buffer_load_b128(r, (int)byte_off, 0, 0);
   return make_uint4(v.x, v.y, v.z, v.w);
+}
+__device__ __forceinline__ unsigned buf_load4(__amdgpu_buffer_rsrc_t r, unsigned byte_off) {
+  return __builtin_amdgcn_raw_buffer_load_b32(r, (int)byte_off, 0, 0);
 }
 
 __device__ __forceinline__ uint4 buf_load16s(__amdgpu_buffer_rsrc_t r, unsigned byte_off, unsigned soff) {
@@ -198,11 +201,15 @@
   int nets, plan_nets;
   long net_ws, net_out0, net_scale;
   int tile_bm, tile_bn;
+  int src_nchw;
+  int w_param;
+  long net_src0, net_w;
 };
 __device__ __forceinline__ ConvParams conv_params_of_net(const ConvParams& pin, int net) {
   ConvParams p = pin;
   if (net != 0) {
-    net_shift(p.src0, p.net_ws); net_shift(p.src1, p.net_ws); net_shift(p.w, p.net_ws);
+    net_shift(p.src0, p.src_nchw ? p.net_src0 : p.net_ws); net_shift(p.src1, p.net_ws);
+    net_shift(p.w, p.w_param ? p.net_w : p.net_ws);
     net_shift(p.out0, p.net_out0); net_shift(p.out1, p.net_ws);
     net_shift(p.stats, p.net_ws); net_shift(p.scale, p.net_scale); net_shift(p.shift, p.net_ws);
     net_shift(p.res, p.net_ws); net_shift(p.partial, p.net_ws);
@@ -337,6 +344,8 @@
   const void* res = nullptr;
   int relu = 0;
   float* slabs = nullptr;
+  const float* src_nchw = nullptr;
+  const float* w_param = nullptr;
 };
 int conv_layer_forward(const ConvLayer& L, const ConvFwdBufs& b, bool wino, hipStream_t s, const NetSplit* ns = nullptr);
 struct ConvDgradBufs {
@@ -351,7 +360,10 @@
   const float* bn_coef = nullptr;
   float* bn_partial = nullptr;
   const void* bn_a = nullptr;
-};
+  const float* dy_nchw = nullptr;
+};
+bool conv_stem_reads_in_place(const ConvLayer& L);
+bool conv_head_dgrad_reads_nchw(const ConvLayer& L);
 int conv_layer_dgrad(const ConvLayer& L, const ConvDgradBufs& b, hipStream_t s, const NetSplit* ns = nullptr);
 struct PackEntry;
 int conv_pack_entry(const ConvLayer& L, long w_off, size_t wf_off, size_t wd_off, bool fwd, bool dgrad, uint32_t block0,
diff --git a/denoising_diffusion_deep_fake_amd/csrc/conv_patch.hip b/denoising_diffusion_deep_fake_amd/csrc/conv_patch.hip
--- a/denoising_diffusion_deep_fake_amd/csrc/conv_patch.hip
+++ b/denoising_diffusion_deep_fake_amd/csrc/conv_patch.hip
@@ -74,6 +74,14 @@
     const int gy = (UP ? y0 / 2 : y0) - 1 + pr, gx = (UP ? x0 / 2 : x0) - 1 + pc;
     const int Hs = UP ? p.H0s : p.Hv, Ws = UP ? p.W0s : p.Wv;
     const bool ok = id < NPV && (unsigned)gy < (unsigned)Hs && (unsigned)gx < (unsigned)Ws;
+    if constexpr (CIN == 4 && !BF) {
+      if (p.src_nchw) {
+        const unsigned plane = (unsigned)(Hs * Ws);
+        const unsigned o = ok ? (unsigned)(b * 3 * Hs * Ws + gy * Ws + gx) * 4u : BUF_OOB;
+        pv[i] = make_uint4(buf_load4(rs, o), buf_load4(rs, o + plane * 4u), buf_load4(rs, o + plane * 8u), 0u);
+        continue;
+      }
+    }
     pv[i] = buf_load16(rs, ok ? (unsigned)(((b * Hs + gy) * Ws + gx) * CSRC + cv * VEC) * (unsigned)sizeof(T) : BUF_OOB);
   }
 #pragma unroll
@@ -469,20 +477,44 @@
   const __amdgpu_buffer_rsrc_t rs = make_rsrc(p.src0, p.src0_bytes);
   const __amdgpu_buffer_rsrc_t rw = make_rsrc(p.w, p.w_bytes);
   uint4 pv[NLP], wv[NLW];
-#pragma unroll
-  for (int i = 0; i < NLP; ++i) {
-    const int id = tid + 256 * i;
-    const int pr = id / PC, pc = id - pr * PC;
-    const int gy = 2 * y0 - 3 + pr, gx = 2 * x0 - 3 + pc;
-    const bool ok = id < NPV && (unsigned)gy < (unsigned)p.Hv && (unsigned)gx < (unsigned)p.Wv;
-    pv[i] = buf_load16(rs, ok ? (unsigned)(((b * p.Hv + gy) * p.Wv + gx) * 4) * 4u : BUF_OOB);
-  }
-#pragma unroll
-  for (int i = 0; i < NLW; ++i) {
-    const int id = tid + 256 * i;
-    const int n = id / 56, r = id - n * 56, kh = r >> 3, kw = r & 7;
-    const bool ok = id < NWV && kw < 7 && (n0 + n) < p.CoutPad;
-    wv[i] = buf_load16(rw, ok ? (unsigned)((n0 + n) * p.w_ld + (kh * 7 + kw) * 4) * 4u : BUF_OOB);
+  if (p.src_nchw) {
+    const int plane = p.Hv * p.Wv;
+#pragma unroll
+    for (int i = 0; i < NLP; ++i) {
+      const int id = tid + 256 * i;
+      const int pr = id / PC, pc = id - pr * PC;
+      const int gy = 2 * y0 - 3 + pr, gx = 2 * x0 - 3 + pc;
+      const bool ok = id < NPV && (unsigned)gy < (unsigned)p.Hv && (unsigned)gx < (unsigned)p.Wv;
+      const unsigned o = ok ? (unsigned)(b * 3 * plane + gy * p.Wv + gx) * 4u : BUF_OOB;
+      pv[i] = make_uint4(buf_load4(rs, o), buf_load4(rs, o + (unsigned)plane * 4u), buf_load4(rs, o + (unsigned)plane * 8u), 0u);
+    }
+  } else {
+#pragma unroll
+    for (int i = 0; i < NLP; ++i) {
+      const int id = tid + 256 * i;
+      const int pr = id / PC, pc = id - pr * PC;
+      const int gy = 2 * y0 - 3 + pr, gx = 2 * x0 - 3 + pc;
+      const bool ok = id < NPV && (unsigned)gy < (unsigned)p.Hv && (unsigned)gx < (unsigned)p.Wv;
+      pv[i] = buf_load16(rs, ok ? (unsigned)(((b * p.Hv + gy) * p.Wv + gx) * 4) * 4u : BUF_OOB);
+    }
+  }
+  if (p.w_param) {
+#pragma unroll
+    for (int i = 0; i < NLW; ++i) {
+      const int id = tid + 256 * i;
+      const int n = id / 56, r = id - n * 56, kh = r >> 3, kw = r & 7;
+      const bool ok = id < NWV && kw < 7 && (n0 + n) < p.Cout;
+      const unsigned o = ok ? (unsigned)((n0 + n) * 147 + kh * 7 + kw) * 4u : BUF_OOB;
+      wv[i] = make_uint4(buf_load4(rw, o), buf_load4(rw, o + 49u * 4u), buf_load4(rw, o + 98u * 4u), 0u);
+    }
+  } else {
+#pragma unroll
+    for (int i = 0; i < NLW; ++i) {
+      const int id = tid + 256 * i;
+      const int n = id / 56, r = id - n * 56, kh = r >> 3, kw = r & 7;
+      const bool ok = id < NWV && kw < 7 && (n0 + n) < p.CoutPad;
+      wv[i] = buf_load16(rw, ok ? (unsigned)((n0 + n) * p.w_ld + (kh * 7 + kw) * 4) * 4u : BUF_OOB);
+    }
   }
 #pragma unroll
   for (int i = 0; i < NLP; ++i) {
diff --git a/denoising_diffusion_deep_fake_amd/csrc/conv_plan.hip b/denoising_diffusion_deep_fake_amd/csrc/conv_plan.hip
--- a/denoising_diffusion_deep_fake_amd/csrc/conv_plan.hip
+++ b/denoising_diffusion_deep_fake_amd/csrc/conv_plan.hip
@@ -132,10 +132,31 @@
   }
 }
 
+bool conv_stem_reads_in_place(const ConvLayer& L) { return L.need_fwd && L.fwd.patch == 2 && L.CinReal == 3 && L.C0 == 4; }
+bool conv_head_dgrad_reads_nchw(const ConvLayer& L) {
+  return L.need_dgrad && !L.upfold && L.dgrad.patch == 1 && L.dgrad.C0 == 4 && L.Cout == 3;
+}
+
 int conv_layer_forward(const ConvLayer& L, const ConvFwdBufs& b, bool wino, hipStream_t s, const NetSplit* ns) {
   ConvParams p = L.fwd;
   p.src0 = b.src0; p.src1 = b.src1; p.w = b.w; p.out0 = b.out;
   net_conv(p, ns);
+  if (b.src_nchw != nullptr || b.w_param != nullptr) {
+    D3F_CHECK(conv_stem_reads_in_place(L) && !wino, "conv: only encoder.conv1's patch kernel reads NCHW input / master weights");
+    if (b.src_nchw != nullptr) {
+      D3F_CHECK((long)L.B * 3 * L.Hv * L.Wv * 4 < (1L << 31), "conv: operand larger than 2 GiB");
+      p.src0 = b.src_nchw;
+      p.src0_bytes = (unsigned)((long)L.B * 3 * L.Hv * L.Wv * 4);
+      p.src_nchw = 1;
+      p.net_src0 = ns != nullptr ? ns->in : 0;
+    }
+    if (b.w_param != nullptr) {
+      p.w = b.w_param;
+      p.w_bytes = (unsigned)((long)L.Cout * 3 * L.KH * L.KW * 4);
+      p.w_param = 1;
+      p.net_w = ns != nullptr ? ns->par : 0;
+    }
+  }
   if (L.head) {
     p.mode = CONV_HEAD_NCHW;
     p.scale = b.bias;
@@ -167,6 +188,14 @@
   p.partial = p.splitk > 1 ? b.slabs : nullptr;
   p.bn_y = b.bn_y; p.bn_coef = b.bn_coef; p.bn_partial = b.bn_partial; p.bn_a = b.bn_a;
   net_conv(p, ns);
+  if (b.dy_nchw != nullptr) {
+    D3F_CHECK(conv_head_dgrad_reads_nchw(L), "conv: only the head's patch data gradient reads an NCHW output gradient");
+    D3F_CHECK((long)L.B * 3 * L.Ho * L.Wo * 4 < (1L << 31), "conv: operand larger than 2 GiB");
+    p.src0 = b.dy_nchw;
+    p.src0_bytes = (unsigned)((long)L.B * 3 * L.Ho * L.Wo * 4);
+    p.src_nchw = 1;
+    p.net_src0 = ns != nullptr ? ns->in : 0;
+  }
   if (p.par == 2 && !p.acc0) {
     const NetSplit nv = net_split_or_single(ns);
     for (int n = 0; n < nv.nets; ++n)
diff --git a/denoising_diffusion_deep_fake_amd/csrc/engine.h b/denoising_diffusion_deep_fake_amd/csrc/engine.h
--- a/denoising_diffusion_deep_fake_amd/csrc/engine.h
+++ b/denoising_diffusion_deep_fake_amd/csrc/engine.h
@@ -139,7 +139,10 @@
   int first_mid_unit_ = -1;
   int first_late_unit_ = -1;
   int forward_body(const float* params, float* bnstats, float* out, char* ws, int training, hipStream_t s,
-                   const NetSplit* ns = nullptr) const;
+                   const NetSplit* ns = nullptr, const float* x_nchw = nullptr) const;
+  bool stem_reads_nchw() const;
+  bool stem_reads_params() const;
+  bool head_dgrad_reads_nchw() const;
   bool make_split(const NetIO* io, long in_delta, NetSplit* ns) const;
   int predict_u8_launches(const float* params, float* bnstats, const uint8_t* bgr_in, uint8_t* bgr_out,
                           const float mean255[3], const float std255[3], char* ws, hipStream_t s) const;
diff --git a/denoising_diffusion_deep_fake_amd/csrc/engine.hip b/denoising_diffusion_deep_fake_amd/csrc/engine.hip
--- a/denoising_diffusion_deep_fake_amd/csrc/engine.hip
+++ b/denoising_diffusion_deep_fake_amd/csrc/engine.hip
@@ -421,6 +421,11 @@
   return 0;
 }
 
+static bool serial_backward() {
+  static const bool serial = getenv("D3F_SERIAL_BACKWARD") != nullptr;
+  return serial;
+}
+
 int UnetEngine::ensure_streams() const {
   if (side_ != nullptr) return 0;
   if (int rc = shared_side_stream(&side_)) return rc;
@@ -442,6 +447,19 @@
   ns->in = in_delta;
   ns->out = io->out;
   return true;
+}
+
+bool UnetEngine::stem_reads_nchw() const {
+  static const bool off = getenv("D3F_NO_STEM_NCHW") != nullptr;
+  return !off && cdtype == D3F_F32 && conv_stem_reads_in_place(units[conv1]);
+}
+bool UnetEngine::stem_reads_params() const {
+  static const bool off = getenv("D3F_NO_STEM_WPARAM") != nullptr;
+  return !off && cdtype == D3F_F32 && conv_stem_reads_in_place(units[conv1]);
+}
+bool UnetEngine::head_dgrad_reads_nchw() const {
+  static const bool off = getenv("D3F_NO_HEAD_NCHW") != nullptr;
+  return !off && cdtype == D3F_F32 && conv_head_dgrad_reads_nchw(units[head]);
 }
 
 int UnetEngine::pack_weights(const float* params0_, void* ws0_, hipStream_t s, const NetIO* io) const {
@@ -463,6 +481,7 @@
       if (first_late_unit_ > 0 && part_of(ui) != part) continue;
       if (first_late_unit_ <= 0 && part != 0) continue;
       if (u.upfold) continue;
+      if (ui == conv1 && stem_reads_params()) continue;
       const int nb = conv_pack_entry(u, u.w_off, u.wf_off, u.wd_off, true, u.need_dgrad, blocks, t.e[t.n++]);
       if (nb < 0) return nb;
       blocks += (uint32_t)nb;
@@ -520,13 +539,19 @@
             "network's offsets");
   NetSplit split{};
   const NetSplit* ns = make_split(io, io ? io->x : 0, &split) ? &split : nullptr;
-  if (int rc = nchw_to_nhwc_launch(dtype, x, ws + tensors[t_x].off, B, in_channels, H, W, tensors[t_x].C, s, ns))
+  const bool direct = training && stem_reads_nchw();
+  if (direct && pack_pending_ && !serial_backward()) {
+    if (int rc = nchw_to_nhwc_launch(dtype, x, ws + tensors[t_x].off, B, in_channels, H, W, tensors[t_x].C, side_, ns))
+      return rc;
+    D3F_HIP(hipEventRecord(ev_pack_done_, side_));
+  } else if (int rc = nchw_to_nhwc_launch(dtype, x, ws + tensors[t_x].off, B, in_channels, H, W, tensors[t_x].C, s, ns)) {
     return rc;
-  return forward_body(params_, bnstats, out, ws, training, s, ns);
+  }
+  return forward_body(params_, bnstats, out, ws, training, s, ns, direct ? x : nullptr);
 }
 
 int UnetEngine::forward_body(const float* params_, float* bnstats, float* out, char* ws, int training,
-                             hipStream_t s, const NetSplit* ns) const {
+                             hipStream_t s, const NetSplit* ns, const float* x_nchw) const {
   auto T = [&](int tid) { return ws + tensors[tid].off; };
   auto coef = [&](const Unit& u) { return reinterpret_cast<float*>(ws + u.coef_off); };
   D3F_CHECK(ns == nullptr || (training && bn_sync() == nullptr), "unet: the pair engine runs train-mode passes with "
@@ -568,6 +593,10 @@
     b.src1 = u.in1 >= 0 ? T(u.in1) : nullptr;
     b.w = ws + (u.wino ? u.wu_off : u.upfold ? u.wfc_off : u.wf_off);
     b.slabs = reinterpret_cast<float*>(ws + splitk_off);
+    if (ui == conv1) {
+      b.src_nchw = x_nchw;
+      if (stem_reads_params()) b.w_param = params_ + u.w_off;
+    }
     if (!u.bn) {
       b.out = out;
       b.bias = params_ + u.bias_off;
@@ -783,10 +812,6 @@
   if (ev_pack_mid_) (void)hipEventDestroy(ev_pack_mid_);
 }
 
-static bool serial_backward() {
-  static const bool serial = getenv("D3F_SERIAL_BACKWARD") != nullptr;
-  return serial;
-}
 
 hipStream_t UnetEngine::side_stream() const {
   if (serial_backward() || ensure_streams() != 0) return nullptr;
@@ -826,9 +851,13 @@
   size_t next_event = 0;
   bool side_used = false;
   constexpr int defer = 3;
+  static const bool no_early_flush = getenv("D3F_NO_EARLY_FLUSH") != nullptr;
+  const int first_flush = no_early_flush ? defer : 2;
   std::vector<int> pending;
   int pending_segment = -1;
   bool head_bias_pending = false;
+  const bool head_direct = head_dgrad_reads_nchw();
+  bool head_dy_pending = false;
   auto flush_pending = [&]() -> int {
     if (pending.empty()) return 0;
     if (!serial) {
@@ -841,6 +870,12 @@
       D3F_HIP(hipStreamWaitEvent(side_, ev_dy_[next_event], 0));
       ++next_event;
       side_used = true;
+    }
+    if (head_dy_pending) {
+      const Unit& uh = units[head];
+      if (int rc = nchw_to_nhwc_launch(dtype, dout, ws + uh.dy_off, B, uh.Cout, uh.Ho, uh.Wo, uh.CoutD, ws_stream, ns))
+        return rc;
+      head_dy_pending = false;
     }
     if (head_bias_pending) {
       const Unit& uh = units[head];
@@ -882,7 +917,11 @@
     const Unit& u = units[op.unit];
     char* dy = ws + u.dy_off;
     if (op.kind == BW_HEAD) {
-      if (int rc = nchw_to_nhwc_launch(dtype, dout, dy, B, u.Cout, u.Ho, u.Wo, u.CoutD, s, ns)) return rc;
+      if (head_direct) {
+        head_dy_pending = !skip_w;
+      } else if (int rc = nchw_to_nhwc_launch(dtype, dout, dy, B, u.Cout, u.Ho, u.Wo, u.CoutD, s, ns)) {
+        return rc;
+      }
       if (skip_w) {
         if (int rc = channel_sum_nchw_launch(dout, B, u.Cout, (long)u.Ho * u.Wo,
                                              reinterpret_cast<float*>(ws + bsum_off), grads + u.bias_off, s, ns))
@@ -903,7 +942,7 @@
     }
     if (!skip_w) {
       pending.push_back(op.unit);
-      if ((int)pending.size() >= defer)
+      if ((int)pending.size() >= (pending.front() == head ? first_flush : defer))
         if (int rc = flush_pending()) return rc;
     }
     if (u.need_dgrad && !skip_d) {
@@ -920,6 +959,7 @@
       d.dx1 = op.dst1 >= 0 ? G(op.dst1) : nullptr;
       d.acc1 = op.acc1 ? 1 : 0;
       d.slabs = reinterpret_cast<float*>(ws + splitk_off);
+      if (op.kind == BW_HEAD && head_direct) d.dy_nchw = dout;
       if (op.fuse_for_unit >= 0) {
         const Unit& uc = units[op.fuse_for_unit];
         d.bn_y = T(uc.y);
diff --git a/denoising_diffusion_deep_fake_amd/ops.py b/denoising_diffusion_deep_fake_amd/ops.py
--- a/denoising_diffusion_deep_fake_amd/ops.py
+++ b/denoising_diffusion_deep_fake_amd/ops.py
@@ -68,6 +68,25 @@
     check(L.d3f_conv_forward(dtype, C.byref(d), ptr(src0), ptr(src1), ptr(wf), ptr(y), ptr(stats), ptr(ws),
                              stream_ptr()))
     return y, stats, tiles.value
+
+
+def conv_stem_forward(d, src0, w, src_nchw=False, w_param=False, want_stats=True):
+    L = _lib.lib()
+    ho, wo = out_hw(d)
+    y = torch.empty((d.B, ho, wo, d.Cout), dtype=torch.float32, device=_dev(src0))
+    tiles = C.c_int()
+    n = L.d3f_conv_stats_floats(F32, C.byref(d), 0, C.byref(tiles))
+    stats = torch.zeros(n, dtype=torch.float32, device=y.device) if want_stats else None
+    check(L.d3f_conv_stem_forward(C.byref(d), ptr(src0.contiguous()), int(src_nchw), ptr(w.contiguous()), int(w_param),
+                                  ptr(y), ptr(stats), stream_ptr()))
+    return y, stats, tiles.value
+
+
+def conv_head_backward_data_nchw(d, dy_nchw, wd):
+    dx0 = torch.empty((d.B, d.H, d.W, d.C0), dtype=torch.float32, device=_dev(dy_nchw))
+    check(_lib.lib().d3f_conv_head_backward_data_nchw(C.byref(d), ptr(dy_nchw.contiguous().float()), ptr(wd), ptr(dx0),
+                                                      stream_ptr()))
+    return dx0
 
 
 def conv_winograd_applies(d, dtype=F32):
diff --git a/include/d3f_hip.h b/include/d3f_hip.h
--- a/include/d3f_hip.h
+++ b/include/d3f_hip.h
@@ -101,6 +101,8 @@
 size_t d3f_conv_stats_floats(int dtype, const d3f_conv_desc* d, int with_workspace, int* tiles);
 int d3f_conv_forward(int dtype, const d3f_conv_desc* d, const void* src0, const void* src1,
                      const void* w_fwd, void* y, float* stats, void* workspace, void* stream);
+int d3f_conv_stem_forward(const d3f_conv_desc* d, const void* src0, int src_is_nchw, const void* w, int w_is_param, void* y,
+                          float* stats, void* stream);
 int d3f_conv_winograd_applies(int dtype, const d3f_conv_desc* d);
 size_t d3f_conv_winograd_filter_bytes(const d3f_conv_desc* d);
 size_t d3f_conv_winograd_stats_floats(const d3f_conv_desc* d, int* tiles);
@@ -111,6 +113,8 @@
 int d3f_conv_upsample_summed(int dtype, const d3f_conv_desc* d);
 int d3f_conv_backward_data(int dtype, const d3f_conv_desc* d, const void* dy, const void* w_dgrad,
                            void* dx0, void* dx1, int acc0, int acc1, void* workspace, void* stream);
+int d3f_conv_head_backward_data_nchw(const d3f_conv_desc* d, const float* dy_nchw, const void* w_dgrad, void* dx0,
+                                     void* stream);
 size_t d3f_conv_backward_weight_workspace_bytes(int dtype, const d3f_conv_desc* d);
 int d3f_conv_backward_weight(int dtype, const d3f_conv_desc* d, const void* dy, const void* src0,
                              const void* src1, void* workspace, float* dw, void* stream);
```

Result: no change. 2046 images/sec (median of 3 runs) (+0.6%).
